# sIncerass/MVLPT

Hardware: AMD Instinct MI355X
Metric: prompt-tuning images/sec (fwd+bwd), ViT-B/16 bs=256, 1/2/4/8 MI355X (higher is better)
Workload: dtype fp16; 1 GPU; BASELINE configs[1]: MVLPT coop head, ViT-B/16, 100 classes (caltech101 token table), n_ctx=16 n_vpt=0, text L=77, class token middle; text_positions_evaluated=77, step_pipelining=True, grad_precision=split_grad, layernorm_folding=both towers, residual_stream=packed fp16 + byte (image tower without prompts / backward), cu_partition=none (towers share every compute unit), per_gpu_batch=256, global_batch=256, parallelism=dp1, text_tower=replicated per GPU

## Files before the change

### include/mvlpt_hip.h

```cpp
#ifndef MVLPT_HIP_H
#define MVLPT_HIP_H
#include <stdint.h>
#ifdef __cplusplus
extern "C" {
#endif

typedef void* mvlpt_stream_t;

enum { MVLPT_DT_F32 = 0, MVLPT_DT_F16 = 1, MVLPT_DT_BF16 = 2 };
enum { MVLPT_LABEL_INT64 = 0, MVLPT_LABEL_PROB_F32 = 1 };
enum { MVLPT_ERR_ARG = -1, MVLPT_ERR_HIP = -2, MVLPT_ERR_STATE = -3, MVLPT_ERR_UNSUPPORTED = -4 };

typedef struct MvlptArch {
  int image_resolution, patch_size, vision_width, vision_layers, vision_heads;
  int context_length, text_width, text_layers, text_heads;
  int embed_dim;
  int compute_dtype;
} MvlptArch;

enum { MVLPT_PREC_FAST = 0, MVLPT_PREC_SPLIT_GRAD = 1, MVLPT_PREC_SPLIT_ALL = 2 };

int mvlpt_create(const MvlptArch* arch, void** handle);
int mvlpt_set_precision(void* handle, int mode);
int mvlpt_set_ln_fold(void* handle, int mode, int min_rows);
// ... 21 lines not shown
                   const int32_t* layout, const int32_t* eot, int C, int L, float* feat_out, int save_for_bwd,
                   mvlpt_stream_t stream);
int mvlpt_text_fwd_grouped(void* handle, const float* prefix, const float* suffix, const float* ctx, int n_ctx, const int32_t* layout,
                           const int32_t* eot, int G, int C, int L, float* feat_out, int save_for_bwd, mvlpt_stream_t stream);
int mvlpt_text_fwd_ranged(void* handle, const float* prefix, const float* suffix, const float* ctx, int n_ctx, const int32_t* layout,
                          const int32_t* eot, const int32_t* class_lo, const int32_t* class_hi, int G, int C, int L, float* feat_out,
                          int save_for_bwd, mvlpt_stream_t stream);
int mvlpt_text_bwd(void* handle, const float* dfeat, float* dctx, mvlpt_stream_t stream);
int mvlpt_text_workspace_bytes(void* handle, int C_total, int L, int save_for_bwd, int64_t* out);

enum { MVLPT_TEXT_MIN_L = 3 };
int mvlpt_text_encode_tokens(void* handle, const int32_t* ids, int ld, int S, int L, float* feat_out, mvlpt_stream_t stream);
int mvlpt_text_ensemble(const float* feats, int T, int C, int e, float* out, mvlpt_stream_t stream);

int mvlpt_logits_fwd(void* handle, const float* img_feat, const float* txt_feat, float logit_scale_exp, const int32_t* task_lo,
                     const int32_t* task_hi, int B, int C, float* logits, mvlpt_stream_t stream);
int mvlpt_logits_bwd(void* handle, const float* dlogits, float* dimg, float* dtxt, mvlpt_stream_t stream);
int mvlpt_logits_grouped_fwd(void* handle, const float* img, const float* txt, float logit_scale_exp, int G, int C, float* logits,
                             mvlpt_stream_t stream);
int mvlpt_logits_grouped_bwd(void* handle, const float* dlogits, float* dtxt, mvlpt_stream_t stream);
int mvlpt_logits_ranged_fwd(void* handle, const float* img, const float* txt, float logit_scale_exp, const int32_t* class_lo,
                            const int32_t* class_hi, int G, int C, float* logits, mvlpt_stream_t stream);
int mvlpt_logits_ranged_bwd(void* handle, const float* dlogits, float* dtxt, float* dimg, mvlpt_stream_t stream);

int mvlpt_cross_entropy(void* handle, const float* logits, const void* labels, int label_kind, int B, int C, float* loss,
                        float* dlogits, float* ncorrect, mvlpt_stream_t stream);

int mvlpt_op_gemm(int dtype, int epi, const void* A, const void* Bt, int M, int N, int K, const float* bias, const void* aux,
                  const float* resid, void* out, void* out2, mvlpt_stream_t stream);
int mvlpt_op_gemm_ex(int dtype, int epi, const void* A, const void* Bt, int M, int N, int K, const float* bias, const void* aux,
                     const float* resid, void* out, void* out2, int a_split, int lda, int ldo, int ldb, int w8_exp, int out_lo8,
                     mvlpt_stream_t stream);
enum { MVLPT_GEMM_BT_128x128_R2 = 1, MVLPT_GEMM_BT_128x128_R4 = 2, MVLPT_GEMM_BT_256x128_R3 = 3, MVLPT_GEMM_BT_256x256_R2 = 4,
       MVLPT_GEMM_PHASED = 5, MVLPT_GEMM_PC = 6, MVLPT_GEMM_PCP = 7 };
int mvlpt_op_gemm_route(int dtype, int epi, int a_split, int M, int N, int K, int fold_ntp, mvlpt_stream_t stream, int* tile_m,
                        int* tile_n, int* ring);
int mvlpt_op_gemm_split(int dtype, int epi, const void* A, const void* Bt, int M, int N, int K, const float* bias, const void* aux,
                        const float* resid, void* out, void* out2, mvlpt_stream_t stream);
int mvlpt_op_layernorm_fwd_split(int out_dtype, const float* x, const float* gamma, const float* beta, void* y, int rows, int d,
                                 mvlpt_stream_t stream);
int mvlpt_op_layernorm_bwd_split(int dtype, const void* dy, const float* x, const float* gamma, const float* resid, float* out32,
                                 void* out16, int rows, int d, mvlpt_stream_t stream);
int mvlpt_op_attention32_fwd(int dtype, const void* qkv, void* out, float* lse, int N, int L, int H, int causal, int q_rows,
                             mvlpt_stream_t stream);
int mvlpt_op_attention32_bwd(int dtype, const void* qkv, const void* out, const void* dout, const float* lse, float* delta,
                             void* dqkv, int N, int L, int H, int causal, mvlpt_stream_t stream);
int mvlpt_op_pack_weight_mixed(int dtype, const float* w32, int rows, int cols, int transposed, void* out, int* w8_exp,
                               mvlpt_stream_t stream);
int mvlpt_op_gemm_mixed(int dtype, int epi, const void* A, const void* Bt, int ldb, int w8_exp, int M, int N, int K, const float* bias,
                        const void* aux, const float* resid, void* out, void* out2, mvlpt_stream_t stream);
int mvlpt_op_cast_mixed(int dtype, const float* in, void* out, int64_t rows, int d, mvlpt_stream_t stream);
int mvlpt_op_fold_vectors(int dtype, const void* W16, int ld, const float* gamma, const float* beta, const float* b, float* colsum,
                          float* bias2, int N, int K, mvlpt_stream_t stream);
int mvlpt_op_gemm_ln_producer(int dtype, const void* A, int a_split, const void* Bt, int ldb, int w8_exp, int M, int N, int K,
                              const float* bias, const float* resid, const float* gamma, int x16_split, float* out32, void* x16,
                              float* part, int ntp, int* nt, mvlpt_stream_t stream);
int mvlpt_op_gemm_folded(int dtype, int epi, const void* A16, int a_split, const void* Bt, int ldb, int w8_exp, int M, int N, int K,
                         const float* colsum, const float* bias2, const float* part, int ntp, int nt, void* out, void* out2,
                         mvlpt_stream_t stream);
int mvlpt_op_fold_weight(const void* W16, int ld, const float* gamma, void* Wg16, int ldg, float* colsum, int N, int K,
                         mvlpt_stream_t stream);
int mvlpt_op_respk_pack(const float* x, void* hi, uint8_t* lo, float* part, int ntp, int rows, int d, mvlpt_stream_t stream);
int mvlpt_op_assemble_packed(const float* patch_emb, const float* cls, const float* pos, const float* ln_g, const float* ln_b, void* hi,
                             uint8_t* lo, float* part, int ntp, int batch, int grid2, int d, mvlpt_stream_t stream);
int mvlpt_op_respk_unpack(const void* hi, const uint8_t* lo, int row_mul, float* out, int rows, int d, mvlpt_stream_t stream);
int mvlpt_op_gemm_residp(const void* A, const void* Bt, int ldb, int M, int N, int K, const float* bias, const void* hi_in,
                         const uint8_t* lo_in, void* hi_out, uint8_t* lo_out, float* part, int ntp, int* nt, mvlpt_stream_t stream);
int mvlpt_op_layernorm_fwd_mixed(int out_dtype, const float* x, const float* gamma, const float* beta, void* y, int rows, int d,
                                 mvlpt_stream_t stream);
int mvlpt_op_layernorm_bwd_mixed(int dtype, const void* dy, const float* x, const float* gamma, const float* resid, float* out32,
                                 void* out16, int rows, int d, mvlpt_stream_t stream);
int mvlpt_op_attention32_fwd_mixed(int dtype, const void* qkv, void* out, float* lse, int N, int L, int H, int causal, int q_rows,
                                   mvlpt_stream_t stream);
int mvlpt_op_attention32_bwd_mixed(int dtype, const void* qkv, const void* out, const void* dout, const float* lse, float* delta,
                                   void* dqkv, int N, int L, int H, int causal, mvlpt_stream_t stream);
int mvlpt_op_layernorm_fwd(int out_dtype, const float* x, const float* gamma, const float* beta, void* y, int rows, int d,
                           mvlpt_stream_t stream);
int mvlpt_op_layernorm_bwd(int dtype, const void* dy, const float* x, const float* gamma, const float* resid, float* out32,
                           void* out16, int rows, int d, mvlpt_stream_t stream);
int mvlpt_op_attention_fwd(int dtype, const void* qkv, void* out, float* lse, int N, int L, int H, int causal,
                           mvlpt_stream_t stream);
int mvlpt_op_attention_bwd(int dtype, const void* qkv, const void* out, const void* dout, const float* lse, float* delta,
                           void* dqkv, int N, int L, int H, int causal, mvlpt_stream_t stream);
int mvlpt_op_cast(int dtype, const float* in, void* out, int64_t n, mvlpt_stream_t stream);
int mvlpt_op_assemble_prompts_grouped(const float* prefix, const float* suffix, const float* ctx, int n_ctx, const int32_t* layout,
                                      const float* pos, float* x, int G, int C, int L, int d, mvlpt_stream_t stream);
int mvlpt_op_gather_ctx_grad_grouped(const float* dx, const int32_t* ctx_pos, int G, int C, int L, int d, int n_ctx, float* dctx,
                                     mvlpt_stream_t stream);
int mvlpt_op_assemble_prompts_ranged(const float* prefix, const float* suffix, const float* ctx, int n_ctx, const int32_t* layout,
                                     const float* pos, float* x, const int32_t* class_lo, const int32_t* class_hi, int G, int C, int L,
                                     int d, mvlpt_stream_t stream);
int mvlpt_op_gather_ctx_grad_ranged(const float* dx, const int32_t* ctx_pos, const int32_t* class_lo, const int32_t* class_hi, int G, int C,
                                    int L, int d, int n_ctx, float* dctx, mvlpt_stream_t stream);

int mvlpt_op_embed_tokens(const float* emb, const float* pos, const int32_t* ids, int ld, float* x, int S, int L, int d,
                          mvlpt_stream_t stream);
int mvlpt_op_ensemble_features(const float* feats, float* out, int T, int C, int e, mvlpt_stream_t stream);
int mvlpt_op_normalize_rows(const float* x, float* xn, float* norm, int rows, int d, mvlpt_stream_t stream);
int mvlpt_op_sgemm_bt(const float* A, const float* Bt, float* C, int M, int N, int K, const float* alpha_dev, mvlpt_stream_t stream);
int mvlpt_op_grad_scale(const float* v, int64_t n, float target, float* scale_dev, mvlpt_stream_t stream);
int mvlpt_op_reduce_prompt_rows(int dtype, float* dx32, void* dx16, int B, int L, int d, int row0, int n, float* out,
                                const float* scale_dev, int zero_after, int split16, const float* vmask, mvlpt_stream_t stream);
int mvlpt_op_gather_ctx_grad(const float* dx, const int32_t* ctx_pos, int C, int L, int d, int n_ctx, int per_class, float* dctx,
                             const float* scale_dev, mvlpt_stream_t stream);
int mvlpt_op_attention_bwd_cls(int dtype, const void* qkv, const void* o_cls, const void* do_cls, const float* lse, void* dqkv, int N,
                               int L, int H, mvlpt_stream_t stream);
int mvlpt_op_copy_rows(const void* src, void* dst, const int32_t* idx, int rows, int row_bytes, int scatter, mvlpt_stream_t stream);
int mvlpt_op_overwrite_rows(const float* rows, int n, float* x, int B, int L, int d, const float* vmask, mvlpt_stream_t stream);
int mvlpt_op_assemble_tokens(const float* patch_emb, const float* cls, const float* pos, const float* ln_g, const float* ln_b,
                             const float* vpt, int n_vpt, const float* vmask, float* x, int B, int G2, int d, mvlpt_stream_t stream);
int mvlpt_op_assemble_prompts(const float* prefix, const float* suffix, const float* ctx, int ctx_per_class, int n_ctx,
                              const int32_t* layout, const float* pos, const int32_t* eot, float* x, int32_t* ctx_pos, int32_t* eot_rows,
                              int C, int L, int d, mvlpt_stream_t stream);

typedef struct MvlptImageDesc {
  int64_t offset;
  int32_t height, width;
  int32_t crop_top, crop_left, crop_height, crop_width;
  int32_t resize_height, resize_width;
  int32_t out_top, out_left;
  int32_t flip;
  int32_t reserved;
} MvlptImageDesc;
int mvlpt_preprocess(void* handle, const uint8_t* src, int64_t src_bytes, const MvlptImageDesc* descs, int B, int out_h, int out_w,
                     const float* mean, const float* std, void* out, int out_dtype, uint8_t* out_u8, mvlpt_stream_t stream);

typedef struct MvlptKernelStat {
  char name[32];
  int64_t launches;
  double ms;
  double flops;
  double bytes;
  double busy_ms;
  double flops_executed;
} MvlptKernelStat;
int mvlpt_profile_begin(void* handle, int all_kernels);
int mvlpt_profile_pause(void* handle, int paused);
int mvlpt_profile_end(void* handle, MvlptKernelStat* stats, int max_stats);

#ifdef __cplusplus
}
#endif
#endif
```

### mvlpt_amd/_lib.py

```python
from __future__ import annotations

import ctypes as C
import os

import torch

_HERE = os.path.dirname(os.path.abspath(__file__))
LIB_PATH = os.environ.get("MVLPT_HIP_LIB") or os.path.join(_HERE, "libmvlpt_hip.so")

DT_F32, DT_F16, DT_BF16 = 0, 1, 2
LABEL_INT64, LABEL_PROB_F32 = 0, 1
EPI_STORE16, EPI_GELU, EPI_RESID32, EPI_GELUBWD, EPI_STORE32, EPI_GELU_SPLIT, EPI_GELUBWD_SPLIT, EPI_STORE_SPLIT = 0, 1, 2, 3, 4, 5, 6, 7
GEMM_BT_128x128_R2, GEMM_BT_128x128_R4, GEMM_BT_256x128_R3, GEMM_BT_256x256_R2, GEMM_PHASED, GEMM_PC, GEMM_PCP = 1, 2, 3, 4, 5, 6, 7
PREC_FAST, PREC_SPLIT_GRAD, PREC_SPLIT_ALL = 0, 1, 2
TEXT_MIN_L = 3


class MvlptArch(C.Structure):
    _fields_ = [(n, C.c_int) for n in (
        "image_resolution", "patch_size", "vision_width", "vision_layers", "vision_heads",
        "context_length", "text_width", "text_layers", "text_heads", "embed_dim", "compute_dtype")]


class MvlptKernelStat(C.Structure):
    _fields_ = [("name", C.c_char * 32), ("launches", C.c_int64), ("ms", C.c_double),
                ("flops", C.c_double), ("bytes", C.c_double), ("busy_ms", C.c_double), ("flops_executed", C.c_double)]


class MvlptImageDesc(C.Structure):
    _fields_ = [("offset", C.c_int64)] + [(n, C.c_int32) for n in (
        "height", "width", "crop_top", "crop_left", "crop_height", "crop_width", "resize_height", "resize_width",
        "out_top", "out_left", "flip", "reserved")]


_vp, _i, _f = C.c_void_p, C.c_int, C.c_float

SIGNATURES = {
    "mvlpt_create": (_i, [C.POINTER(MvlptArch), C.POINTER(_vp)]),
    "mvlpt_destroy": (_i, [_vp]),
    "mvlpt_set_precision": (_i, [_vp, _i]),
    "mvlpt_trim": (_i, [_vp]),
    "mvlpt_debug_checksums": (_i, [_vp, _i, C.POINTER(C.c_uint64), _i]),
    "mvlpt_set_ln_fold": (_i, [_vp, _i, _i]),
    "mvlpt_set_resid_packed": (_i, [_vp, _i]),
    "mvlpt_set_vpt_dropout": (_i, [_vp, _vp, _i, _i, _i, _i]),
    "mvlpt_last_error": (C.c_char_p, [_vp]),
    "mvlpt_version": (C.c_char_p, []),
    "mvlpt_stream_create_cus": (_i, [_i, _i, C.POINTER(_vp)]),
    "mvlpt_stream_destroy": (_i, [_vp]),
    "mvlpt_stream_cus": (_i, [_vp]),
    "mvlpt_load_frozen": (_i, [_vp, C.c_char_p, _vp, _i, C.POINTER(C.c_int64), _i, _vp]),
    "mvlpt_frozen_ready": (_i, [_vp]),
    "mvlpt_image_fwd": (_i, [_vp, _vp, _i, _vp, _vp, _i, _i, _i, _vp, _i, _vp]),
    "mvlpt_image_bwd": (_i, [_vp, _vp, _vp, _vp, _vp]),
    "mvlpt_text_fwd": (_i, [_vp, _vp, _vp, _vp, _i, _i, _vp, _vp, _i, _i, _vp, _i, _vp]),
    "mvlpt_text_bwd": (_i, [_vp, _vp, _vp, _vp]),
    "mvlpt_text_fwd_grouped": (_i, [_vp, _vp, _vp, _vp, _i, _vp, _vp, _i, _i, _i, _vp, _i, _vp]),
    "mvlpt_text_fwd_ranged": (_i, [_vp, _vp, _vp, _vp, _i, _vp, _vp, _vp, _vp, _i, _i, _i, _vp, _i, _vp]),
    "mvlpt_text_workspace_bytes": (_i, [_vp, _i, _i, _i, C.POINTER(C.c_int64)]),
    "mvlpt_text_encode_tokens": (_i, [_vp, _vp, _i, _i, _i, _vp, _vp]),
    "mvlpt_text_ensemble": (_i, [_vp, _i, _i, _i, _vp, _vp]),
    "mvlpt_logits_fwd": (_i, [_vp, _vp, _vp, _f, _vp, _vp, _i, _i, _vp, _vp]),
    "mvlpt_logits_bwd": (_i, [_vp, _vp, _vp, _vp, _vp]),
    "mvlpt_logits_grouped_fwd": (_i, [_vp, _vp, _vp, _f, _i, _i, _vp, _vp]),
    "mvlpt_logits_grouped_bwd": (_i, [_vp, _vp, _vp, _vp]),
    "mvlpt_logits_ranged_fwd": (_i, [_vp, _vp, _vp, _f, _vp, _vp, _i, _i, _vp, _vp]),
    "mvlpt_logits_ranged_bwd": (_i, [_vp, _vp, _vp, _vp, _vp]),
    "mvlpt_cross_entropy": (_i, [_vp, _vp, _vp, _i, _i, _i, _vp, _vp, _vp, _vp]),
    "mvlpt_op_gemm": (_i, [_i, _i, _vp, _vp, _i, _i, _i, _vp, _vp, _vp, _vp, _vp, _vp]),
    "mvlpt_op_gemm_ex": (_i, [_i, _i, _vp, _vp, _i, _i, _i, _vp, _vp, _vp, _vp, _vp, _i, _i, _i, _i, _i, _i, _vp]),
    "mvlpt_op_gemm_route": (_i, [_i, _i, _i, _i, _i, _i, _i, _vp, C.POINTER(_i), C.POINTER(_i), C.POINTER(_i)]),
    "mvlpt_op_gemm_split": (_i, [_i, _i, _vp, _vp, _i, _i, _i, _vp, _vp, _vp, _vp, _vp, _vp]),
    "mvlpt_op_layernorm_fwd_split": (_i, [_i, _vp, _vp, _vp, _vp, _i, _i, _vp]),
    "mvlpt_op_layernorm_bwd_split": (_i, [_i, _vp, _vp, _vp, _vp, _vp, _vp, _i, _i, _vp]),
    "mvlpt_op_attention32_fwd": (_i, [_i, _vp, _vp, _vp, _i, _i, _i, _i, _i, _vp]),
    "mvlpt_op_attention32_bwd": (_i, [_i, _vp, _vp, _vp, _vp, _vp, _vp, _i, _i, _i, _i, _vp]),
    "mvlpt_op_pack_weight_mixed": (_i, [_i, _vp, _i, _i, _i, _vp, C.POINTER(C.c_int), _vp]),
    "mvlpt_op_gemm_mixed": (_i, [_i, _i, _vp, _vp, _i, _i, _i, _i, _i, _vp, _vp, _vp, _vp, _vp, _vp]),
    "mvlpt_op_cast_mixed": (_i, [_i, _vp, _vp, C.c_int64, _i, _vp]),
    "mvlpt_op_fold_vectors": (_i, [_i, _vp, _i, _vp, _vp, _vp, _vp, _vp, _i, _i, _vp]),
    "mvlpt_op_gemm_ln_producer": (_i, [_i, _vp, _i, _vp, _i, _i, _i, _i, _i, _vp, _vp, _vp, _i, _vp, _vp, _vp, _i, C.POINTER(C.c_int), _vp]),
    "mvlpt_op_gemm_folded": (_i, [_i, _i, _vp, _i, _vp, _i, _i, _i, _i, _i, _vp, _vp, _vp, _i, _i, _vp, _vp, _vp]),
    "mvlpt_op_fold_weight": (_i, [_vp, _i, _vp, _vp, _i, _vp, _i, _i, _vp]),
    "mvlpt_op_respk_pack": (_i, [_vp, _vp, _vp, _vp, _i, _i, _i, _vp]),
    "mvlpt_op_assemble_packed": (_i, [_vp, _vp, _vp, _vp, _vp, _vp, _vp, _vp, _i, _i, _i, _i, _vp]),
    "mvlpt_op_respk_unpack": (_i, [_vp, _vp, _i, _vp, _i, _i, _vp]),
    "mvlpt_op_gemm_residp": (_i, [_vp, _vp, _i, _i, _i, _i, _vp, _vp, _vp, _vp, _vp, _vp, _i, C.POINTER(C.c_int), _vp]),
    "mvlpt_op_layernorm_fwd_mixed": (_i, [_i, _vp, _vp, _vp, _vp, _i, _i, _vp]),
    "mvlpt_op_layernorm_bwd_mixed": (_i, [_i, _vp, _vp, _vp, _vp, _vp, _vp, _i, _i, _vp]),
    "mvlpt_op_attention32_fwd_mixed": (_i, [_i, _vp, _vp, _vp, _i, _i, _i, _i, _i, _vp]),
    "mvlpt_op_attention32_bwd_mixed": (_i, [_i, _vp, _vp, _vp, _vp, _vp, _vp, _i, _i, _i, _i, _vp]),
    "mvlpt_op_layernorm_fwd": (_i, [_i, _vp, _vp, _vp, _vp, _i, _i, _vp]),
    "mvlpt_op_layernorm_bwd": (_i, [_i, _vp, _vp, _vp, _vp, _vp, _vp, _i, _i, _vp]),
    "mvlpt_op_attention_fwd": (_i, [_i, _vp, _vp, _vp, _i, _i, _i, _i, _vp]),
    "mvlpt_op_attention_bwd": (_i, [_i, _vp, _vp, _vp, _vp, _vp, _vp, _i, _i, _i, _i, _vp]),
    "mvlpt_op_cast": (_i, [_i, _vp, _vp, C.c_int64, _vp]),
    "mvlpt_op_assemble_prompts_grouped": (_i, [_vp, _vp, _vp, _i, _vp, _vp, _vp, _i, _i, _i, _i, _vp]),
    "mvlpt_op_gather_ctx_grad_grouped": (_i, [_vp, _vp, _i, _i, _i, _i, _i, _vp, _vp]),
    "mvlpt_op_assemble_prompts_ranged": (_i, [_vp, _vp, _vp, _i, _vp, _vp, _vp, _vp, _vp, _i, _i, _i, _i, _vp]),
    "mvlpt_op_gather_ctx_grad_ranged": (_i, [_vp, _vp, _vp, _vp, _i, _i, _i, _i, _i, _vp, _vp]),
    "mvlpt_op_embed_tokens": (_i, [_vp, _vp, _vp, _i, _vp, _i, _i, _i, _vp]),
    "mvlpt_op_ensemble_features": (_i, [_vp, _vp, _i, _i, _i, _vp]),
    "mvlpt_op_normalize_rows": (_i, [_vp, _vp, _vp, _i, _i, _vp]),
    "mvlpt_op_sgemm_bt": (_i, [_vp, _vp, _vp, _i, _i, _i, _vp, _vp]),
    "mvlpt_op_grad_scale": (_i, [_vp, C.c_int64, _f, _vp, _vp]),
    "mvlpt_op_reduce_prompt_rows": (_i, [_i, _vp, _vp, _i, _i, _i, _i, _i, _vp, _vp, _i, _i, _vp, _vp]),
    "mvlpt_op_gather_ctx_grad": (_i, [_vp, _vp, _i, _i, _i, _i, _i, _vp, _vp, _vp]),
    "mvlpt_op_attention_bwd_cls": (_i, [_i, _vp, _vp, _vp, _vp, _vp, _i, _i, _i, _vp]),
    "mvlpt_op_copy_rows": (_i, [_vp, _vp, _vp, _i, _i, _i, _vp]),
    "mvlpt_op_overwrite_rows": (_i, [_vp, _i, _vp, _i, _i, _i, _vp, _vp]),
    "mvlpt_op_assemble_tokens": (_i, [_vp, _vp, _vp, _vp, _vp, _vp, _i, _vp, _vp, _i, _i, _i, _vp]),
    "mvlpt_op_assemble_prompts": (_i, [_vp, _vp, _vp, _i, _i, _vp, _vp, _vp, _vp, _vp, _vp, _i, _i, _i, _vp]),
    "mvlpt_preprocess": (_i, [_vp, _vp, C.c_int64, C.POINTER(MvlptImageDesc), _i, _i, _i, C.POINTER(_f), C.POINTER(_f), _vp, _i, _vp, _vp]),
    "mvlpt_profile_begin": (_i, [_vp, _i]),
    "mvlpt_profile_pause": (_i, [_vp, _i]),
    "mvlpt_profile_end": (_i, [_vp, C.POINTER(MvlptKernelStat), _i]),
}


def load_library(path: str = LIB_PATH) -> C.CDLL:
    if not os.path.isfile(path):
        raise ImportError(
            f"{path} not found: build the HIP extension first (`make` at the repo root, or "
            "`__graft_entry__.build()`); mvlpt_amd has no CPU fallback.")
    lib = C.CDLL(path)
    for name, (res, args) in SIGNATURES.items():
        fn = getattr(lib, name)
        fn.restype, fn.argtypes = res, args
    return lib


lib = load_library()


def last_error(handle=None) -> str:
    msg = lib.mvlpt_last_error(handle)
    return msg.decode() if msg else ""


def check(rc: int, handle=None, what: str = "") -> None:
    if rc != 0:
        raise RuntimeError(f"libmvlpt_hip {what} failed (code {rc}): {last_error(handle) or last_error(None)}")
```

### mvlpt_amd/csrc/attention.hip

```cpp
#include <hip/hip_ext.h>
#include "attn_common.h"

namespace mvlpt {

constexpr int ATT_MAX_NKT = 38;
int attn_max_len() { return ATT_MAX_NKT * 16; }

template <typename T, int NKT, bool CAUSAL>
__global__ __launch_bounds__(256) void attn_fwd_kernel(AttnArgs a) {
  extern __shared__ __attribute__((aligned(16))) char smem[];
  using v8 = typename Vec<T>::v8;
  using v4 = typename Vec<T>::v4;
  constexpr int LP = NKT * 16;
  constexpr int BLK = NKT < 16 ? NKT : 16;
  constexpr bool PRELOAD = NKT <= 16;
  char* sK = smem;
  char* sV = smem + LP * 128;
  const int L = a.L, H = a.H, d = H * 64;
  const int n = blockIdx.x / H, h = blockIdx.x % H;
  const size_t ld = (size_t)3 * d;
  const T* base = (const T*)a.qkv + (size_t)n * L * ld + h * 64;
  const int lane = threadIdx.x & 63, wave = __builtin_amdgcn_readfirstlane(threadIdx.x >> 6);
  const int fr = lane & 15, fg = lane >> 4;
  const int nqt = a.q_rows > 0 ? ((a.q_rows < L ? a.q_rows : L) + 15) >> 4 : (L + 15) >> 4;
// ... 480 lines not shown
template <typename T>
__device__ __forceinline__ float cls_dot16(const float* g16, const typename Vec<T>::v8& a0, const typename Vec<T>::v8& a1) {
  float s = 0.f;
#pragma unroll
  for (int e = 0; e < 8; ++e) { s = fmaf(g16[e], to_f32<T>(a0[e]), s); s = fmaf(g16[e + 8], to_f32<T>(a1[e]), s); }
  s += __shfl_xor(s, 1, 64); s += __shfl_xor(s, 2, 64);
  return s;
}
template <typename T>
__global__ __launch_bounds__(256) void attn_bwd_cls_kernel(const T* __restrict__ qkv, const T* __restrict__ o_cls,
                                                           const T* __restrict__ do_cls, const float* __restrict__ lse,
                                                           T* __restrict__ dqkv, int N, int L, int H) {
  using v8 = typename Vec<T>::v8;
  __shared__ float sq[64], sdo[64], red[4][64];
  const int n = blockIdx.x / H, h = blockIdx.x % H, d = H * 64, tid = threadIdx.x;
  const size_t ld = (size_t)3 * d;
  const T* base = qkv + (size_t)n * L * ld + h * 64;
  T* gbase = dqkv + (size_t)n * L * ld + h * 64;
  if (tid < 64) {
    sq[tid] = to_f32<T>(base[tid]);
    sdo[tid] = to_f32<T>(do_cls[(size_t)n * d + h * 64 + tid]);
  }
  __syncthreads();
  const float l0 = lse[((size_t)n * H + h) * L];
  const int lane = tid & 63, wave = tid >> 6, kg = lane >> 2, ch = lane & 3;
  float q16[16], g16[16], dqa[16];
#pragma unroll
  for (int e = 0; e < 16; ++e) { q16[e] = sq[ch * 16 + e]; g16[e] = sdo[ch * 16 + e]; dqa[e] = 0.f; }
  const T* op = o_cls + (size_t)n * d + h * 64 + ch * 16;
  const float delta = cls_dot16<T>(g16, *(const v8*)op, *(const v8*)(op + 8));
  for (int j0 = wave * 16; j0 < L; j0 += 64) {
    const int j = j0 + kg;
    const int jc = j < L ? j : L - 1;
    const T* kp = base + (size_t)jc * ld + d + ch * 16;
    const v8 k0 = *(const v8*)kp, k1 = *(const v8*)(kp + 8);
    const v8 v0 = *(const v8*)(kp + d), v1 = *(const v8*)(kp + d + 8);
    float k16[16], sdot = 0.f;
#pragma unroll
    for (int e = 0; e < 8; ++e) { k16[e] = to_f32<T>(k0[e]); k16[e + 8] = to_f32<T>(k1[e]); }
    const float dp = cls_dot16<T>(g16, v0, v1);
#pragma unroll
    for (int e = 0; e < 16; ++e) sdot += q16[e] * k16[e];
    sdot += __shfl_xor(sdot, 1, 64); sdot += __shfl_xor(sdot, 2, 64);
    const float pj = j < L ? __expf(sdot * 0.125f - l0) : 0.f;
    const float ds = pj * (dp - delta) * 0.125f;
    v8 wk[2], wv[2], wz[2];
#pragma unroll
    for (int e = 0; e < 16; ++e) {
      dqa[e] += ds * k16[e];
      wk[e >> 3][e & 7] = from_f32<T>(ds * q16[e]);
      wv[e >> 3][e & 7] = from_f32<T>(pj * g16[e]);
      wz[e >> 3][e & 7] = from_f32<T>(0.f);
    }
    if (j < L) {
      T* gp = gbase + (size_t)j * ld + ch * 16;
      if (j > 0) { *(v8*)gp = wz[0]; *(v8*)(gp + 8) = wz[1]; }
      *(v8*)(gp + d) = wk[0]; *(v8*)(gp + d + 8) = wk[1];
      *(v8*)(gp + 2 * d) = wv[0]; *(v8*)(gp + 2 * d + 8) = wv[1];
    }
  }
#pragma unroll
  for (int e = 0; e < 16; ++e) {
    float v = dqa[e];
    v += __shfl_xor(v, 4, 64); v += __shfl_xor(v, 8, 64); v += __shfl_xor(v, 16, 64); v += __shfl_xor(v, 32, 64);
    if (kg == 0) red[wave][ch * 16 + e] = v;
  }
  __syncthreads();
  if (tid < 64) gbase[tid] = from_f32<T>(red[0][tid] + red[1][tid] + red[2][tid] + red[3][tid]);
}

hipError_t launch_attn_bwd_cls(int dtype, const void* qkv, const void* o_cls, const void* do_cls, const float* lse, void* dqkv,
                               int N, int L, int H, hipStream_t s) {
  if (N <= 0 || L <= 0 || H <= 0) return hipErrorInvalidValue;
  if (dtype == DT_F16)
    hipLaunchKernelGGL(attn_bwd_cls_kernel<f16>, dim3(N * H), dim3(256), 0, s, (const f16*)qkv, (const f16*)o_cls, (const f16*)do_cls, lse,
                       (f16*)dqkv, N, L, H);
  else if (dtype == DT_BF16)
    hipLaunchKernelGGL(attn_bwd_cls_kernel<bf16>, dim3(N * H), dim3(256), 0, s, (const bf16*)qkv, (const bf16*)o_cls, (const bf16*)do_cls,
                       lse, (bf16*)dqkv, N, L, H);
  else return hipErrorInvalidValue;
  return hipGetLastError();
}

static thread_local hipEvent_t t_ev_a = nullptr, t_ev_b = nullptr;
template <typename T, int NKT, bool CAUSAL>
static hipError_t fwd_t(const AttnArgs& a, hipStream_t s) {
  constexpr int LP = NKT * 16;
  constexpr int lds = 2 * LP * 128;
  static bool set = false;
  if (!set) { hipFuncSetAttribute((const void*)attn_fwd_kernel<T, NKT, CAUSAL>, hipFuncAttributeMaxDynamicSharedMemorySize, lds); set = true; }
  hipExtLaunchKernelGGL((attn_fwd_kernel<T, NKT, CAUSAL>), dim3(a.N * a.H), dim3(256), lds, s, t_ev_a, t_ev_b, 0, a);
  return hipGetLastError();
}
template <typename T, int NKT, bool CAUSAL>
static hipError_t bwd_t(const AttnBwdArgs& a, hipStream_t s) {
  constexpr int LP = NKT * 16;
  constexpr int lds_a = 2 * LP * 128;
  constexpr int lds_b = 2 * LP * 128 + 2 * LP * 4;
  static bool set = false;
  if (!set) {
    hipFuncSetAttribute((const void*)attn_bwd_dq_kernel<T, NKT, CAUSAL>, hipFuncAttributeMaxDynamicSharedMemorySize, lds_a);
    hipFuncSetAttribute((const void*)attn_bwd_dkv_kernel<T, NKT, CAUSAL>, hipFuncAttributeMaxDynamicSharedMemorySize, lds_b);
    set = true;
  }
  hipLaunchKernelGGL((attn_bwd_dq_kernel<T, NKT, CAUSAL>), dim3(a.N * a.H), dim3(256), lds_a, s, a);
  hipError_t e = hipGetLastError();
  if (e != hipSuccess) return e;
  hipLaunchKernelGGL((attn_bwd_dkv_kernel<T, NKT, CAUSAL>), dim3(a.N * a.H), dim3(256), lds_b, s, a);
  return hipGetLastError();
}

#define MVLPT_NKT_SWITCH(FN, ARGS)                                  \
  switch (nkt) {                                                    \
    case 2: return FN<T, 2, CAUSAL> ARGS;                           \
    case 4: return FN<T, 4, CAUSAL> ARGS;                           \
    case 6: return FN<T, 6, CAUSAL> ARGS;                           \
    case 8: return FN<T, 8, CAUSAL> ARGS;                           \
    case 10: return FN<T, 10, CAUSAL> ARGS;                         \
    case 12: return FN<T, 12, CAUSAL> ARGS;                         \
    case 14: return FN<T, 14, CAUSAL> ARGS;                         \
    case 16: return FN<T, 16, CAUSAL> ARGS;                         \
  }                                                                 \
  if constexpr (!CAUSAL) {    \
    if (nkt == 18) return FN<T, 18, CAUSAL> ARGS;                   \
    if (nkt == 38) return FN<T, 38, CAUSAL> ARGS;                   \
  }                                                                 \
  return hipErrorInvalidValue;

template <typename T, bool CAUSAL> static hipError_t fwd_n(int nkt, const AttnArgs& a, hipStream_t s) {
  if constexpr (!CAUSAL) { if (nkt == 13) return fwd_t<T, 13, CAUSAL>(a, s); }
  MVLPT_NKT_SWITCH(fwd_t, (a, s))
}
template <typename T, bool CAUSAL> static hipError_t bwd_n(int nkt, const AttnBwdArgs& a, hipStream_t s) { MVLPT_NKT_SWITCH(bwd_t, (a, s)) }

static int nkt_for(int L) {
  int t = (L + 15) / 16; t += t & 1;
  if (t > 18) return 38;
  return t < 2 ? 2 : t;
}

static bool use_stream(int L) { return L > 256; }

hipError_t launch_attn_fwd(int dtype, const AttnArgs& a_, hipStream_t s, hipEvent_t ea, hipEvent_t eb) {
  t_ev_a = ea; t_ev_b = eb;
  AttnArgs a = a_;
  a.flags = 3;
  if (a.L <= 0 || a.L > attn_max_len() || a.N <= 0) return hipErrorInvalidValue;
  if (use_stream(a.L)) return launch_attn_fwd_stream(dtype, a, s);
  if (!a.causal && a.q_rows <= 0 && (a.L + 15) / 16 == PNT && (dtype == DT_F16 || dtype == DT_BF16)) {
    const int total = a.N * a.H, cus = stream_cus(s);
    if (total >= 2 * cus) {
      static bool set = false;
      if (!set) {
        hipFuncSetAttribute((const void*)attn_fwdp_kernel<f16>, hipFuncAttributeMaxDynamicSharedMemorySize, PLDS);
        hipFuncSetAttribute((const void*)attn_fwdp_kernel<bf16>, hipFuncAttributeMaxDynamicSharedMemorySize, PLDS);
        set = true;
      }
      if (dtype == DT_F16) hipExtLaunchKernelGGL((attn_fwdp_kernel<f16>), dim3(cus), dim3(PNW * 64), PLDS, s, ea, eb, 0, a, total);
      else hipExtLaunchKernelGGL((attn_fwdp_kernel<bf16>), dim3(cus), dim3(PNW * 64), PLDS, s, ea, eb, 0, a, total);
      return hipGetLastError();
    }
  }
  const int nkt = !a.causal && (a.L + 15) / 16 == 13 ? 13 : nkt_for(a.L);
  if (dtype == DT_F16) return a.causal ? fwd_n<f16, true>(nkt, a, s) : fwd_n<f16, false>(nkt, a, s);
  if (dtype == DT_BF16) return a.causal ? fwd_n<bf16, true>(nkt, a, s) : fwd_n<bf16, false>(nkt, a, s);
  return hipErrorInvalidValue;
// ... 12 lines not shown
```

### mvlpt_amd/csrc/attention32.hip

```cpp
#include "attn_common.h"

namespace mvlpt {

#ifdef MVLPT_ATTN_TRACE
constexpr int ATR_MAX = 256;
#define MVLPT_ATR(p) do { if (a.trace && blockIdx.x == 1024 && lane == 0 && atr_n < ATR_MAX) \
    a.trace[wave * ATR_MAX + atr_n++] = ((long long)(p) << 56) | ((long long)__builtin_amdgcn_s_memtime() & 0xffffffffffffffLL); } while (0)
#define MVLPT_ATRB(p) do { if (a.trace && blockIdx.x == 5 && blockIdx.y == (gridDim.y >> 1) && lane == 0 && atr_n < ATR_MAX) \
    a.trace[wave * ATR_MAX + atr_n++] = ((long long)(p) << 56) | ((long long)__builtin_amdgcn_s_memtime() & 0xffffffffffffffLL); } while (0)
#else
#define MVLPT_ATR(p) do { } while (0)
#define MVLPT_ATRB(p) do { } while (0)
#endif

namespace {
constexpr int CH = 64;
constexpr int XIMG = CH * 128;
constexpr float SCALE = 0.125f;

template <typename T>
__device__ __forceinline__ void store_pair4(T* p, size_t lo_off, f32x4 v) {
  typename Vec<T>::v4 hi, lo;
#pragma unroll
  for (int e = 0; e < 4; ++e) { T h, l; split16<T>(v[e], h, l); hi[e] = h; lo[e] = l; }
// ... 1094 lines not shown
static bool attn32_resident(int L, int causal) { return !causal && L <= RROWS; }

static int attn32_nw(int rows) {
  const int pad8 = (rows + 255) / 256 * 256, pad4 = (rows + 127) / 128 * 128;
  return pad8 * 8 <= pad4 * 9 ? 8 : 4;
}
template <typename K>
static void set_lds(K kernel, int bytes) { (void)hipFuncSetAttribute((const void*)kernel, hipFuncAttributeMaxDynamicSharedMemorySize, bytes); }

template <typename T, bool CAUSAL, int NW>
static hipError_t fwd_x(const Attn32Args& a, hipStream_t s) {
  const int lq = a.q_rows > 0 ? (a.q_rows < a.L ? a.q_rows : a.L) : a.L;
  const int nqc = (lq + NW * 32 - 1) / (NW * 32);
  constexpr int lds = 8 * XIMG;
  static bool set = false;
  if (!set) { set_lds(attn32x_fwd_kernel<T, CAUSAL, NW>, lds); set = true; }
  hipLaunchKernelGGL((attn32x_fwd_kernel<T, CAUSAL, NW>), dim3(stream_grid(a.N * a.H, nqc)), dim3(NW * 64), lds, s, a, nqc);
  return hipGetLastError();
}
template <typename T, bool CAUSAL, int NW>
static hipError_t bwd_x(const Attn32BwdArgs& a, hipStream_t s) {
  const int nc = (a.L + NW * 32 - 1) / (NW * 32), lpad = (a.L + CH - 1) / CH * CH;
  constexpr int lds = 8 * XIMG;
  const int lds_kv = lds + 8 * lpad;
  static int set = 0;
  if (set < lds_kv) {
    set_lds(attn32x_dq_kernel<T, CAUSAL, NW>, lds); set_lds(attn32x_dkv_kernel<T, CAUSAL, NW>, lds_kv);
    set_lds(attn32x_bwd_fused_kernel<T, CAUSAL, NW>, lds_kv); set = lds_kv;
  }
  const dim3 grid(stream_grid(a.N * a.H, nc)), block(NW * 64);
  if (nc == 1) {
    hipLaunchKernelGGL((attn32x_bwd_fused_kernel<T, CAUSAL, NW>), grid, block, lds_kv, s, a, lpad);
    return hipGetLastError();
  }
  hipLaunchKernelGGL((attn32x_dq_kernel<T, CAUSAL, NW>), grid, block, lds, s, a, nc);
  hipLaunchKernelGGL((attn32x_dkv_kernel<T, CAUSAL, NW>), grid, block, lds_kv, s, a, nc, lpad);
  return hipGetLastError();
}

template <typename T>
static hipError_t fwd_t(const Attn32Args& a, hipStream_t s) {
  if (a.L <= SROWS) {
    dim3 grid(a.H, a.N), block(SNT * 64);
    if (a.causal) hipLaunchKernelGGL((attn32t_fwd_kernel<T, true>), grid, block, 0, s, a);
    else hipLaunchKernelGGL((attn32t_fwd_kernel<T, false>), grid, block, 0, s, a);
    return hipGetLastError();
  }
  if (attn32_resident(a.L, a.causal)) {
    const int total = a.N * a.H, cus = stream_cus(s);
    if (a.q_rows <= 0 && total >= 2 * cus) {
      static bool setp = false;
      if (!setp) { set_lds(attn32p_fwd_kernel<T>, RLDS_P); setp = true; }
      hipLaunchKernelGGL((attn32p_fwd_kernel<T>), dim3(cus), dim3(RNW * 64), RLDS_P, s, a, total);
      return hipGetLastError();
    }
    static bool set = false;
    if (!set) { set_lds(attn32r_fwd_kernel<T>, RLDS); set = true; }
    hipLaunchKernelGGL((attn32r_fwd_kernel<T>), dim3(a.H, a.N), dim3(RNW * 64), RLDS, s, a);
    return hipGetLastError();
  }
  const int lq = a.q_rows > 0 ? (a.q_rows < a.L ? a.q_rows : a.L) : a.L;
  if (attn32_nw(lq) == 8) return a.causal ? fwd_x<T, true, 8>(a, s) : fwd_x<T, false, 8>(a, s);
  return a.causal ? fwd_x<T, true, 4>(a, s) : fwd_x<T, false, 4>(a, s);
}
template <typename T>
static hipError_t bwd_t(const Attn32BwdArgs& a, hipStream_t s) {
  if (a.L <= SROWS) {
    dim3 grid(a.H, a.N), block(SNT * 64);
    if (a.causal) hipLaunchKernelGGL((attn32t_bwd_kernel<T, true>), grid, block, 0, s, a);
    else hipLaunchKernelGGL((attn32t_bwd_kernel<T, false>), grid, block, 0, s, a);
    return hipGetLastError();
  }
  if (attn32_resident(a.L, a.causal)) {
    static bool set = false;
    if (!set) { set_lds(attn32r_bwd_kernel<T>, RLDS_BWD); set = true; }
    hipLaunchKernelGGL((attn32r_bwd_kernel<T>), dim3(a.H, a.N), dim3(RNW * 64), RLDS_BWD, s, a);
    return hipGetLastError();
  }
  if (a.L > 8192) return hipErrorInvalidValue;
  if (attn32_nw(a.L) == 8) return a.causal ? bwd_x<T, true, 8>(a, s) : bwd_x<T, false, 8>(a, s);
  return a.causal ? bwd_x<T, true, 4>(a, s) : bwd_x<T, false, 4>(a, s);
}

hipError_t launch_attn32_fwd(int dtype, const Attn32Args& a, hipStream_t s) {
  if (a.L <= 0 || a.N <= 0 || a.H <= 0 || !a.qkv_split || !a.out_split) return hipErrorInvalidValue;
  if (dtype == DT_F16) return fwd_t<f16>(a, s);
  if (dtype == DT_BF16) return fwd_t<bf16>(a, s);
  return hipErrorInvalidValue;
}
hipError_t launch_attn32_bwd(int dtype, const Attn32BwdArgs& a, hipStream_t s) {
  if (a.L <= 0 || a.N <= 0 || a.H <= 0 || !a.qkv_split || !a.out_split || !a.dout_split || !a.lse || !a.delta || !a.dqkv_split)
    return hipErrorInvalidValue;
  if (dtype == DT_F16) return bwd_t<f16>(a, s);
  if (dtype == DT_BF16) return bwd_t<bf16>(a, s);
  return hipErrorInvalidValue;
}

}
```

### mvlpt_amd/csrc/engine.hip

```cpp
#include <hip/hip_runtime.h>

#include <cmath>
#include <cstdio>
#include <algorithm>
#include <array>
#include <map>
#include <cstring>
#include <mutex>
#include <string>
#include <vector>

#include "../../include/mvlpt_hip.h"
#include "kernels.h"

using namespace mvlpt;


namespace {
struct StreamPart { hipStream_t s; int cus; };
std::mutex g_part_mu;
std::vector<StreamPart> g_parts;
int device_cus() {
  static int cus = 0;
  if (!cus) {
// ... 32 lines not shown
  }
  hipError_t reserve(size_t bytes) {
    if (bytes <= cap) return hipSuccess;
    size_t got = std::max(bytes, cap + cap / 2);
    void* q = nullptr;
    hipError_t e = hipMalloc(&q, got);
    if (e != hipSuccess && got > bytes) { got = bytes; e = hipMalloc(&q, got); }
    if (e != hipSuccess) return e;
    if (p) retired.push_back(p);
    p = q; cap = got;
    return hipSuccess;
  }
};
struct Bump {
  char* base = nullptr; size_t off = 0, cap = 0;
  template <typename T> T* take(size_t count) {
    size_t bytes = (count * sizeof(T) + 255) & ~(size_t)255;
    T* r = (T*)(base + off); off += bytes; return r;
  }
  void* take_bytes(size_t bytes) { return take<char>(bytes); }
};
static size_t align256(size_t b) { return (b + 255) & ~(size_t)255; }

struct WRef { const void* p; int ld; int e8; };
struct Linear {
  void* w = nullptr; void* wt = nullptr; float* b = nullptr; int out = 0, in = 0;
  int ldw = 0, ldwt = 0, e8 = 0;
  float *fold_s = nullptr, *fold_b = nullptr;
  void* wg = nullptr; float* fold_sg = nullptr;
  WRef fw() const { return WRef{w, ldw, e8}; }
  WRef fwg() const { return WRef{wg, in, 0}; }
  WRef bw() const { return WRef{wt, ldwt, e8}; }
};
struct LNp { float* g = nullptr; float* b = nullptr; };
struct Block { LNp ln1, ln2; Linear qkv, o, fc, pr; };
struct TowerW { int width = 0, layers = 0, heads = 0; std::vector<Block> blocks; };

struct TowerState {
  bool valid = false, saved = false, causal = false;
  bool exact = false;
  int wide_pitch = 0;
  int xs = 0;
  int N = 0, L = 0, d = 0, H = 0, layers = 0;
  std::vector<float*> x;
  std::vector<void*> qkv, attn, u;
  std::vector<float*> lse;
  void *h16 = nullptr, *a16 = nullptr;
  float* dx32 = nullptr; void *dx16 = nullptr, *du16 = nullptr, *dO16 = nullptr, *dqkv16 = nullptr; float* dh32 = nullptr;
  float* delta = nullptr; float* scale_dev = nullptr;
  std::vector<char> skip;
  bool fold = false;
  float* part[2] = {nullptr, nullptr};
  int nt[2] = {0, 0}, ntp[2] = {0, 0};
};
constexpr int FOLD_NTP = 8;

enum ProfClass { PC_GEMM = 0, PC_ATTN_FWD, PC_ATTN_BWD, PC_LN_FWD, PC_LN_BWD, PC_GLUE, PC_HEAD, PC_ATTN_FWD_IMG, PC_COUNT };
static const char* kProfNames[PC_COUNT] = {"gemm_bt", "attention_fwd", "attention_bwd", "layernorm_fwd", "layernorm_bwd",
                                           "glue", "head_logits_ce", "attention_fwd_image"};
struct ProfRec { int cls; hipEvent_t a, b; double flops, bytes, flops_exec; int M = 0, N = 0, K = 0, epi = -1, split = 0, fold = 0; };

struct Engine {
  MvlptArch arch{};
  int dt = DT_F16;
  int prec_mode = MVLPT_PREC_SPLIT_GRAD;
  int fold_mode = 2;
  int fold_min_rows = 1024;
  bool fold_ready = false;
  int resid_packed = 1;
  const float* vpt_mask = nullptr;
  int vpt_mask_layers = 0, vpt_mask_B = 0, vpt_mask_n = 0, vpt_mask_d = 0;
  const float* v_mask = nullptr;
  bool lo8 = true;
  std::string err;
  TowerW vis, txt;
  void* conv_w = nullptr; int Kp = 0; float* cls_emb = nullptr; float* vpos = nullptr; LNp ln_pre, ln_post;
  float *vproj = nullptr, *vproj_t = nullptr;
  float* tpos = nullptr; LNp ln_final; float *tproj = nullptr, *tproj_t = nullptr;
  float* tok_emb = nullptr; int vocab = 0;
  std::vector<void*> owned;
  DevBuf vis_ws, txt_ws, head_ws, ce_ws, tmp, pp_ws;
  TowerState vs, ts;
  int vB = 0, v_nvpt = 0, v_ndeep = 0; float* cls32 = nullptr; float* dcls32 = nullptr;
  float* xc32 = nullptr; void *ac16 = nullptr, *hc16 = nullptr, *gc16 = nullptr;
  bool v_cls_last = false; float *xcm32 = nullptr, *xco32 = nullptr, *dxc32 = nullptr, *dhc32 = nullptr;
  void *uc16 = nullptr, *duc16 = nullptr, *dxc16 = nullptr, *dOc16 = nullptr;
  int tC = 0, tL = 0, t_nctx = 0, t_per_class = 0; int32_t* eot_rows = nullptr; int32_t* ctx_pos = nullptr;
  int t_groups = 0, t_gC = 0;
  bool t_ranged = false; const int32_t *t_rlo = nullptr, *t_rstart = nullptr;
  std::vector<int32_t> t_range_host, h_range_host;
  std::vector<int32_t> t_ids_host;
  bool t_eot_last = false; float *txc32 = nullptr, *txm32 = nullptr, *txo32 = nullptr, *tdxc32 = nullptr, *tdhc32 = nullptr;
  void *tac16 = nullptr, *thc16 = nullptr, *tgc16 = nullptr, *tuc16 = nullptr, *tduc16 = nullptr, *tdxc16 = nullptr, *tdOc16 = nullptr;
  float* eot32 = nullptr; float* deot32 = nullptr;
  int hB = 0, hC = 0; float h_scale = 0.f; const int32_t *h_lo = nullptr, *h_hi = nullptr;
  bool h_grouped = false;
  bool h_ranged = false; int hS = 0; const int32_t *h_rlo = nullptr, *h_rstart = nullptr, *h_rgrp = nullptr;
  float *imn = nullptr, *txn = nullptr, *inorm = nullptr, *tnorm = nullptr;
  unsigned long long* dbg_ck = nullptr; int dbg_ck_n = 0; bool dbg_ck_on = false;
  bool prof_on = false, prof_all = false; std::vector<ProfRec> prof; std::vector<hipEvent_t> ev_pool; size_t ev_used = 0;
};

thread_local std::string g_create_err;

int fail(Engine* E, int code, const std::string& msg) { if (E) E->err = msg; else g_create_err = msg; return code; }
int hipfail(Engine* E, hipError_t e, const char* what) {
  return fail(E, MVLPT_ERR_HIP, std::string(what) + ": " + hipGetErrorString(e));
}
#define HIPCHK(E, call) do { hipError_t _e = (call); if (_e != hipSuccess) return hipfail((E), _e, #call); } while (0)

struct ProfScope {
  Engine* E; hipStream_t s; bool on = false; hipEvent_t b{};
  ProfScope(Engine* E_, hipStream_t s_, int cls, double flops, double bytes) : E(E_), s(s_) {
    if (!E || !E->prof_on || !E->prof_all) return;
    if (E->ev_used + 2 > E->ev_pool.size()) {
      if (E->ev_pool.size() >= 65536) return;
      for (int i = 0; i < 512; ++i) { hipEvent_t ev; if (hipEventCreate(&ev) != hipSuccess) return; E->ev_pool.push_back(ev); }
    }
    hipEvent_t a = E->ev_pool[E->ev_used++]; b = E->ev_pool[E->ev_used++];
    (void)hipEventRecord(a, s);
    E->prof.push_back(ProfRec{cls, a, b, flops, bytes, flops});
    on = true;
  }
  ~ProfScope() { if (on) (void)hipEventRecord(b, s); }
};

constexpr int DBG_CK_MAX = 256;
static void dbg_ck(Engine* E, const void* p, size_t bytes, hipStream_t s) {
  if (!E->dbg_ck_on || !E->dbg_ck || E->dbg_ck_n >= DBG_CK_MAX) return;
  (void)launch_checksum(p, bytes, E->dbg_ck + E->dbg_ck_n++, s);
}

static hipError_t attn_fwd_timed(Engine* E, const AttnArgs& a, double flops, double bytes, hipStream_t s) {
  hipEvent_t ea = nullptr, eb = nullptr;
  if (E && E->prof_on && !E->prof_all) {
    if (E->ev_used + 2 > E->ev_pool.size() && E->ev_pool.size() < 65536)
      for (int i = 0; i < 512; ++i) { hipEvent_t ev; if (hipEventCreate(&ev) != hipSuccess) break; E->ev_pool.push_back(ev); }
    if (E->ev_used + 2 <= E->ev_pool.size()) {
      ea = E->ev_pool[E->ev_used++]; eb = E->ev_pool[E->ev_used++];
      E->prof.push_back(ProfRec{PC_ATTN_FWD_IMG, ea, eb, flops, bytes, flops});
    }
  }
  return launch_attn_fwd(E->dt, a, s, ea, eb);
}

struct Fold {
  const float* ln_gamma = nullptr; void* ln_x16 = nullptr; int ln_split = 0; float* ln_part = nullptr; int ln_ntp = 0;
  const float* fold_part = nullptr; const float* fold_colsum = nullptr; int fold_ntp = 0, fold_nt = 0;
  const void* rp_hi_in = nullptr; const uint8_t* rp_lo_in = nullptr; uint8_t* rp_lo_out = nullptr;
};
hipError_t gemm(Engine* E, int epi, const void* A, WRef Bt, int M, int N, int K, const float* bias, const void* aux,
                const float* resid, void* out, void* out2, hipStream_t s, int dtype = -1, int a_split = 0, const Fold* f = nullptr,
                int lda = 0, int ldo = 0) {
  GemmArgs g{A, Bt.p, M, N, K, bias, aux, resid, out, out2};
  g.a_split = a_split; g.ldb = Bt.ld; g.w8_exp = Bt.e8; g.lda = lda; g.ldo = ldo;
  if (f) {
    g.ln_gamma = f->ln_gamma; g.ln_x16 = f->ln_x16; g.ln_split = f->ln_split; g.ln_part = f->ln_part; g.ln_ntp = f->ln_ntp;
    g.fold_part = f->fold_part; g.fold_colsum = f->fold_colsum; g.fold_ntp = f->fold_ntp; g.fold_nt = f->fold_nt;
    g.rp_hi_in = f->rp_hi_in; g.rp_lo_in = f->rp_lo_in; g.rp_lo_out = f->rp_lo_out;
  }
  g.out_lo8 = (a_split == 2 && (epi == EPI_GELU_SPLIT || epi == EPI_GELUBWD_SPLIT)) ? 1 : 0;
  const int dt = dtype >= 0 ? dtype : E->dt;
  const double ob = (epi == EPI_RESIDP_LN) ? 6.0 : (epi == EPI_RESID32) ? 8.0 : (epi == EPI_RESID32_LN) ? 8.0 + 2.0 * (a_split ? 1.5 : 1.0) : ((epi == EPI_STORE32 || epi == EPI_STORE_SPLIT) ? 4.0 : ((epi == EPI_GELUBWD || epi == EPI_GELU_SPLIT) ? 4.0 :
                    (epi == EPI_GELUBWD_SPLIT ? 6.0 : 2.0)));
  hipEvent_t ea = nullptr, eb = nullptr;
  if (E && E->prof_on) {
    if (E->ev_used + 2 > E->ev_pool.size() && E->ev_pool.size() < 65536)
// ... 506 lines not shown
  const MvlptArch& A = E->arch;
  const int dv = A.vision_width, dtw = A.text_width, e = A.embed_dim;
  const int G2 = (A.image_resolution / A.patch_size) * (A.image_resolution / A.patch_size);
  auto is1 = [&](int r) { return ndim == 1 && shape[0] == r; };
  auto is2 = [&](int r, int c) { return ndim == 2 && shape[0] == r && shape[1] == c; };
  int rc = 0;
  const char* vb = "visual.transformer.resblocks.";
  const char* tb = "transformer.resblocks.";
  if (nm.rfind(vb, 0) == 0 || nm.rfind(tb, 0) == 0) {
    const bool isv = nm.rfind(vb, 0) == 0;
    int layer; const char* tail;
    if (!parse_block_name(name + strlen(isv ? vb : tb), &layer, &tail)) return fail(E, MVLPT_ERR_ARG, "malformed block name: " + nm);
    rc = load_block_tensor(E, isv ? E->vis : E->txt, layer, tail, p32, shape, ndim, s);
  } else if (nm == "visual.conv1.weight") {
    if (!(ndim == 4 && shape[0] == dv && shape[1] == 3 && shape[2] == A.patch_size && shape[3] == A.patch_size))
      return fail(E, MVLPT_ERR_ARG, "shape mismatch: " + nm);
    void* w = nullptr;
    HIPCHK(E, hipMalloc(&w, (size_t)dv * E->Kp * 2)); E->owned.push_back(w);
    HIPCHK(E, launch_pack_weight(E->dt, p32, w, dv, 3 * A.patch_size * A.patch_size, E->Kp, s));
    E->conv_w = w;
  } else if (nm == "visual.class_embedding") { if (!is1(dv)) return fail(E, MVLPT_ERR_ARG, "shape mismatch: " + nm); rc = upload_f32(E, p32, n, &E->cls_emb, s);
  } else if (nm == "visual.positional_embedding") { if (!is2(G2 + 1, dv)) return fail(E, MVLPT_ERR_ARG, "shape mismatch: " + nm); rc = upload_f32(E, p32, n, &E->vpos, s);
  } else if (nm == "visual.ln_pre.weight") { if (!is1(dv)) return fail(E, MVLPT_ERR_ARG, "shape mismatch: " + nm); rc = upload_f32(E, p32, n, &E->ln_pre.g, s);
  } else if (nm == "visual.ln_pre.bias") { if (!is1(dv)) return fail(E, MVLPT_ERR_ARG, "shape mismatch: " + nm); rc = upload_f32(E, p32, n, &E->ln_pre.b, s);
  } else if (nm == "visual.ln_post.weight") { if (!is1(dv)) return fail(E, MVLPT_ERR_ARG, "shape mismatch: " + nm); rc = upload_f32(E, p32, n, &E->ln_post.g, s);
  } else if (nm == "visual.ln_post.bias") { if (!is1(dv)) return fail(E, MVLPT_ERR_ARG, "shape mismatch: " + nm); rc = upload_f32(E, p32, n, &E->ln_post.b, s);
  } else if (nm == "visual.proj") {
    if (!is2(dv, e)) return fail(E, MVLPT_ERR_ARG, "shape mismatch: " + nm);
    void *w = nullptr, *wt = nullptr;
    HIPCHK(E, hipMalloc(&w, n * 4)); E->owned.push_back(w);
    HIPCHK(E, hipMalloc(&wt, n * 4)); E->owned.push_back(wt);
    HIPCHK(E, launch_pack_weight(DT_F32, p32, w, dv, e, e, s));
    HIPCHK(E, launch_pack_weight_t(DT_F32, p32, wt, dv, e, s));
    E->vproj = (float*)w; E->vproj_t = (float*)wt;
  } else if (nm == "positional_embedding") { if (!is2(A.context_length, dtw)) return fail(E, MVLPT_ERR_ARG, "shape mismatch: " + nm); rc = upload_f32(E, p32, n, &E->tpos, s);
  } else if (nm == "ln_final.weight") { if (!is1(dtw)) return fail(E, MVLPT_ERR_ARG, "shape mismatch: " + nm); rc = upload_f32(E, p32, n, &E->ln_final.g, s);
  } else if (nm == "ln_final.bias") { if (!is1(dtw)) return fail(E, MVLPT_ERR_ARG, "shape mismatch: " + nm); rc = upload_f32(E, p32, n, &E->ln_final.b, s);
  } else if (is_tok) {
    if (!(ndim == 2 && shape[0] > 0 && shape[0] <= INT32_MAX && shape[1] == dtw)) return fail(E, MVLPT_ERR_ARG, "shape mismatch: " + nm);
    E->vocab = 0;
    rc = upload_f32(E, p32, n, &E->tok_emb, s);
    if (!rc) E->vocab = (int)shape[0];
  } else if (nm == "text_projection") {
    if (!is2(dtw, e)) return fail(E, MVLPT_ERR_ARG, "shape mismatch: " + nm);
    void *w = nullptr, *wt = nullptr;
    HIPCHK(E, hipMalloc(&w, n * 4)); E->owned.push_back(w);
    HIPCHK(E, hipMalloc(&wt, n * 4)); E->owned.push_back(wt);
    HIPCHK(E, launch_pack_weight(DT_F32, p32, w, dtw, e, e, s));
    HIPCHK(E, launch_pack_weight_t(DT_F32, p32, wt, dtw, e, s));
    E->tproj = (float*)w; E->tproj_t = (float*)wt;
  } else {
    return fail(E, MVLPT_ERR_ARG, "unknown frozen tensor name: " + nm);
  }
  if (rc) return rc;
  if (dtype != MVLPT_DT_F32) HIPCHK(E, hipStreamSynchronize(s));
  return 0;
}

int mvlpt_frozen_ready(void* h) {
  Engine* E = (Engine*)h;
  if (!E) return MVLPT_ERR_ARG;
  const char* m = first_missing(E);
  if (m) return fail(E, MVLPT_ERR_STATE, std::string("frozen tensor not loaded: ") + m);
  return 0;
}

int mvlpt_image_fwd(void* h, const void* image, int image_dtype, const float* vpt, const float* vpt_deep, int n_vpt, int n_deep,
                    int B, float* feat_out, int save_for_bwd, mvlpt_stream_t stream) {
  Engine* E = (Engine*)h;
  if (!E || !image || !feat_out || B <= 0) return fail(E, MVLPT_ERR_ARG, "image_fwd: null/invalid argument");
  if (int rc = mvlpt_frozen_ready(h)) return rc;
  if ((n_vpt > 0) != (vpt != nullptr)) return fail(E, MVLPT_ERR_ARG, "image_fwd: vpt pointer and n_vpt disagree");
  if ((n_deep > 0) != (vpt_deep != nullptr) || (n_deep > 0 && n_vpt <= 0)) return fail(E, MVLPT_ERR_ARG, "image_fwd: deep prompts need vpt");
  hipStream_t s = (hipStream_t)stream;
  const MvlptArch& A = E->arch;
  const int G = A.image_resolution / A.patch_size, G2 = G * G, dv = A.vision_width, e = A.embed_dim;
  const int Lv = 1 + n_vpt + G2;
  if (Lv > attn_max_len()) return fail(E, MVLPT_ERR_UNSUPPORTED, "image_fwd: sequence length > 256 not supported yet");
  const bool save = save_for_bwd != 0;
  const bool exact = E->prec_mode == MVLPT_PREC_SPLIT_ALL || (E->prec_mode == MVLPT_PREC_SPLIT_GRAD && save);
  const size_t X = exact ? 2 : 1;
  const size_t npatch = (size_t)B * G2;
  size_t need = tower_bytes(E->vis, B, Lv, save, exact) + align256(npatch * E->Kp * 2) + align256(npatch * dv * 4) +
                7 * align256((size_t)B * dv * 4) + 4 * align256((size_t)B * dv * 2 * X) + 3 * align256((size_t)B * dv * 8 * X) + 4096;
  E->vs.valid = false;
  HIPCHK(E, E->vis_ws.reserve(need));
  Bump bp; bp.base = (char*)E->vis_ws.p; bp.cap = E->vis_ws.cap;
  void* patches = bp.take_bytes(npatch * E->Kp * 2);
  float* pe = bp.take<float>(npatch * dv);
  E->cls32 = bp.take<float>((size_t)B * dv);
  E->dcls32 = bp.take<float>((size_t)B * dv);
  E->xc32 = bp.take<float>((size_t)B * dv);
  E->ac16 = bp.take_bytes((size_t)B * dv * 2 * X); E->hc16 = bp.take_bytes((size_t)B * dv * 2 * X);
  E->gc16 = bp.take_bytes((size_t)B * dv * 4 * 2 * X);
  E->xcm32 = bp.take<float>((size_t)B * dv); E->xco32 = bp.take<float>((size_t)B * dv);
  E->dxc32 = bp.take<float>((size_t)B * dv); E->dhc32 = bp.take<float>((size_t)B * dv);
  E->dxc16 = bp.take_bytes((size_t)B * dv * 2 * X); E->dOc16 = bp.take_bytes((size_t)B * dv * 2 * X);
  E->uc16 = bp.take_bytes((size_t)B * dv * 4 * 2); E->duc16 = bp.take_bytes((size_t)B * dv * 4 * 2 * X);
  E->v_cls_last = false;
  carve_tower(bp, E->vis, E->vs, B, Lv, save, false, exact, split_kind(E));
  TowerState& st = E->vs;
  E->vB = B; E->v_nvpt = n_vpt; E->v_ndeep = n_deep;
  st.fold = E->fold_mode >= 1 && (size_t)B * Lv >= (size_t)E->fold_min_rows && dv >= 256;
  if (st.fold) if (int rc = prepare_fold(E, s)) return rc;

  const float* const masks = E->vpt_mask;
  const int mask_layers = E->vpt_mask_layers, mask_B = E->vpt_mask_B, mask_n = E->vpt_mask_n;
  E->vpt_mask = nullptr; E->vpt_mask_layers = 0; E->v_mask = nullptr;
  if (masks && (n_vpt <= 0 || mask_layers < 1 + n_deep || mask_B != B || mask_n != n_vpt))
    return fail(E, MVLPT_ERR_ARG, "image_fwd: the prompt dropout masks do not match this forward (layers >= 1 + n_deep, batch, n_vpt)");
  E->v_mask = masks;
  auto vmask = [&](int l) -> const float* { return masks ? masks + (size_t)l * B * n_vpt * dv : nullptr; };
  { ProfScope ps(E, s, PC_GLUE, 0, (double)npatch * E->Kp * 6.0);
    HIPCHK(E, launch_patchify(E->dt, image, image_dtype, patches, B, A.image_resolution, A.patch_size, E->Kp, s)); }
  if (E->dbg_ck_on) { E->dbg_ck_n = 0; if (E->dbg_ck) (void)hipMemsetAsync(E->dbg_ck, 0, DBG_CK_MAX * sizeof(unsigned long long), s); }
  dbg_ck(E, patches, (size_t)npatch * E->Kp * 2, s);
  HIPCHK(E, gemm(E, EPI_STORE32, patches, WRef{E->conv_w, 0, 0}, (int)npatch, dv, E->Kp, nullptr, nullptr, nullptr, pe, nullptr, s));
  dbg_ck(E, pe, (size_t)npatch * dv * 4, s);
  const int nt_d = dv / 128, ntp_d = (nt_d + 1) & ~1;
  const bool packed = E->resid_packed && E->dt == DT_F16 && !save && !exact && st.fold && n_vpt == 0 && dv % 128 == 0 &&
                      ntp_d <= FOLD_NTP && E->vis.blocks[0].qkv.wg != nullptr;
  void* const xhi = st.x[0];
  uint8_t* const xlo = (uint8_t*)st.x[0] + (size_t)B * Lv * dv * 2;
  if (packed) {
    ProfScope ps(E, s, PC_GLUE, 0, (double)B * Lv * dv * 7.0);
    HIPCHK(E, launch_assemble_tokens_packed(pe, E->cls_emb, E->vpos, E->ln_pre.g, E->ln_pre.b, xhi, xlo, st.part[0], ntp_d, B, G2, dv, s));
    st.nt[0] = nt_d; st.ntp[0] = ntp_d;
    dbg_ck(E, xhi, (size_t)B * Lv * dv * 3, s); dbg_ck(E, st.part[0], (size_t)B * Lv * ntp_d * 8, s);
  } else {
    ProfScope ps(E, s, PC_GLUE, 0, (double)B * Lv * dv * 8.0);
    HIPCHK(E, launch_assemble_tokens(pe, E->cls_emb, E->vpos, E->ln_pre.g, E->ln_pre.b, vpt, n_vpt, st.x[0], B, G2, dv, s, vmask(0)));
  }
  bool cls_only_last = false;
  bool ln1_ready = packed;
  auto next_foldable = [&](int l) -> const LNp* {
    const int n = l + 1;
    if (!st.fold || n >= E->vis.layers) return nullptr;
    if (n_deep > 0) return nullptr;
    return &E->vis.blocks[n].ln1;
  };
  for (int l = 0; l < E->vis.layers; ++l) {
    if (l > 0 && n_deep > 0) {
      if (l <= n_deep) {
        ProfScope ps(E, s, PC_GLUE, 0, (double)B * n_vpt * dv * 4.0);
        HIPCHK(E, launch_overwrite_rows(vpt_deep + (size_t)(l - 1) * n_vpt * dv, n_vpt, st.x[2 * l], B, Lv, dv, s, vmask(l)));
      } else {
        st.skip[l] = 1;
        if (st.saved) {
          HIPCHK(E, hipMemcpyAsync(st.x[2 * l + 2], st.x[2 * l], (size_t)B * Lv * dv * 4, hipMemcpyDeviceToDevice, s));
        }
        continue;
      }
    }
    if (l == E->vis.layers - 1) { cls_only_last = true; break; }
    if (packed) { if (int rc = block_fwd_packed(E, E->vis, st, l, s)) return rc; continue; }
    bool produced = false;
    if (int rc = block_fwd(E, E->vis, st, l, s, ln1_ready, next_foldable(l), &produced)) return rc;
    ln1_ready = produced;
  }
  if (cls_only_last) {
    const int l = E->vis.layers - 1;
    const Block& Bk = E->vis.blocks[l];
    const int T = B * Lv;
    float* xin = st.x[2 * l];
    float* xmid = save ? E->xcm32 : E->xc32;
    float* xout = save ? E->xco32 : E->xc32;
    E->v_cls_last = save;
    const int xs = st.xs;
    Fold fq;
    if (ln1_ready) fq = fold_consumer(st, 0, Bk.qkv);
    else HIPCHK(E, ln_fwd(E, E->dt, xin, nullptr, 1, Bk.ln1, st.h16, T, dv, s, xs));
    if (packed) fq.fold_colsum = Bk.qkv.fold_sg;
    HIPCHK(E, gemm(E, xs ? EPI_STORE_SPLIT : EPI_STORE16, packed ? xhi : st.h16, packed ? Bk.qkv.fwg() : Bk.qkv.fw(), T, 3 * dv, dv,
                   ln1_ready ? Bk.qkv.fold_b : Bk.qkv.b, nullptr, nullptr, st.qkv[l], nullptr, s, -1, xs, ln1_ready ? &fq : nullptr));
    dbg_ck(E, st.qkv[l], (size_t)T * 3 * dv * 2 * X, s);
    if (xs) {
      if (save) HIPCHK(E, launch_zero(st.attn[l], (size_t)T * dv * 4, s));
      if (int rc = attn32_fwd(E, st, l, 1, s)) return rc;
    } else {
      AttnArgs a{st.qkv[l], st.attn[l], save ? st.lse[l] : nullptr, st.N, st.L, st.H, 0, 1};
      ProfScope ps(E, s, PC_ATTN_FWD, 4.0 * st.L * 64.0 * st.N * st.H, (double)T * dv * 2.0 * 2.0);
      HIPCHK(E, launch_attn_fwd(E->dt, a, s));
    }
    { ProfScope ps(E, s, PC_GLUE, 0, (double)B * dv * 12.0);
      HIPCHK(E, launch_copy_rows_strided(st.attn[l], E->ac16, B, (size_t)Lv * dv * 2 * X, (size_t)dv * 2 * X, (int)(dv * 2 * X), s));
      if (packed) HIPCHK(E, launch_respk_unpack_rows(xhi, xlo, Lv, E->xc32, B, dv, s));
      else HIPCHK(E, launch_copy_rows_strided(xin, E->xc32, B, (size_t)Lv * dv * 4, (size_t)dv * 4, dv * 4, s)); }
    dbg_ck(E, E->ac16, (size_t)B * dv * 2 * X, s); dbg_ck(E, E->xc32, (size_t)B * dv * 4, s);
    HIPCHK(E, gemm(E, EPI_RESID32, E->ac16, Bk.o.fw(), B, dv, dv, Bk.o.b, nullptr, E->xc32, xmid, nullptr, s, -1, xs));
    HIPCHK(E, ln_fwd(E, E->dt, xmid, nullptr, 1, Bk.ln2, E->hc16, B, dv, s, xs));
    HIPCHK(E, gemm(E, xs ? EPI_GELU_SPLIT : EPI_GELU, E->hc16, Bk.fc.fw(), B, 4 * dv, dv, Bk.fc.b, nullptr, nullptr, E->gc16, save ? E->uc16 : nullptr, s, -1, xs));
    HIPCHK(E, gemm(E, EPI_RESID32, E->gc16, Bk.pr.fw(), B, dv, 4 * dv, Bk.pr.b, nullptr, xmid, xout, nullptr, s, -1, xs));
    HIPCHK(E, ln_fwd(E, DT_F32, xout, nullptr, 1, E->ln_post, E->cls32, B, dv, s));
  } else
  HIPCHK(E, ln_fwd(E, DT_F32, st.x[2 * E->vis.layers], nullptr, Lv, E->ln_post, E->cls32, B, dv, s));
  { ProfScope ps(E, s, PC_HEAD, 2.0 * B * e * dv, 4.0 * ((double)B * dv + (double)e * dv + (double)B * e));
    HIPCHK(E, launch_sgemm_bt(E->cls32, E->vproj_t, feat_out, B, e, dv, nullptr, s)); }
  return 0;
}

int mvlpt_image_bwd(void* h, const float* dfeat, float* dvpt, float* dvpt_deep, mvlpt_stream_t stream) {
  Engine* E = (Engine*)h;
  if (!E || !dfeat) return fail(E, MVLPT_ERR_ARG, "image_bwd: null argument");
  TowerState& st = E->vs;
  if (!st.valid || !st.saved) return fail(E, MVLPT_ERR_STATE, "image_bwd: call image_fwd(save_for_bwd=1) first");
  if ((E->v_nvpt > 0 && !dvpt) || (E->v_ndeep > 0 && !dvpt_deep)) return fail(E, MVLPT_ERR_ARG, "image_bwd: missing gradient output");
  hipStream_t s = (hipStream_t)stream;
  const MvlptArch& A = E->arch;
  const int B = E->vB, dv = A.vision_width, e = A.embed_dim, Lv = st.L, n = E->v_nvpt;
  const size_t T = (size_t)B * Lv;
  { ProfScope ps(E, s, PC_GLUE, 0, (double)T * dv * 10.0);
    HIPCHK(E, launch_grad_scale(dfeat, (size_t)B * e, 64.0f, st.scale_dev, s));
    HIPCHK(E, launch_sgemm_bt(dfeat, E->vproj, E->dcls32, B, dv, e, st.scale_dev, s)); }
  { ProfScope ps(E, s, PC_GLUE, 0, (double)T * dv * 4.0);
    HIPCHK(E, launch_zero(st.dx32, T * dv * 4, s)); }
  int l_top = st.layers - 1;
  const int xs = st.xs;
  if (E->v_cls_last) {
    const int l = st.layers - 1;
    const Block& Bk = E->vis.blocks[l];
    const int Ti = (int)T;
    HIPCHK(E, ln_bwd(E, E->dcls32, DT_F32, E->xco32, nullptr, 1, E->ln_post, nullptr, E->dxc32, E->dxc16, B, dv, s, -1, xs));
    HIPCHK(E, gemm(E, xs ? EPI_GELUBWD_SPLIT : EPI_GELUBWD, E->dxc16, Bk.pr.bw(), B, 4 * dv, dv, nullptr, E->uc16, nullptr, E->duc16, nullptr, s, -1, xs));
    HIPCHK(E, gemm(E, EPI_STORE32, E->duc16, Bk.fc.bw(), B, dv, 4 * dv, nullptr, nullptr, nullptr, E->dhc32, nullptr, s, -1, xs));
    HIPCHK(E, ln_bwd(E, E->dhc32, DT_F32, E->xcm32, nullptr, 1, Bk.ln2, E->dxc32, E->dxc32, E->dxc16, B, dv, s, -1, xs));
    HIPCHK(E, gemm(E, xs ? EPI_STORE_SPLIT : EPI_STORE16, E->dxc16, Bk.o.bw(), B, dv, dv, nullptr, nullptr, nullptr, E->dOc16, nullptr, s, -1, xs));
    if (xs) {
      { ProfScope ps(E, s, PC_GLUE, 0, (double)T * dv * 4.0);
        HIPCHK(E, launch_zero(st.dO16, T * dv * 4, s));
        HIPCHK(E, launch_copy_rows_strided(E->dOc16, st.dO16, B, (size_t)dv * 4, (size_t)Lv * dv * 4, dv * 4, s)); }
      if (int rc = attn32_bwd(E, st, l, s)) return rc;
    } else {
      ProfScope ps(E, s, PC_ATTN_BWD, 10.0 * st.L * 64.0 * st.N * st.H, (double)T * dv * 2.0 * 5.0);
      HIPCHK(E, launch_attn_bwd_cls(E->dt, st.qkv[l], E->ac16, E->dOc16, st.lse[l], st.dqkv16, st.N, st.L, st.H, s)); }
    { ProfScope ps(E, s, PC_GLUE, 0, (double)B * dv * 8.0);
      HIPCHK(E, launch_copy_rows_strided(E->dxc32, st.dx32, B, (size_t)dv * 4, (size_t)Lv * dv * 4, dv * 4, s)); }
    HIPCHK(E, gemm(E, EPI_STORE32, st.dqkv16, Bk.qkv.bw(), Ti, dv, 3 * dv, nullptr, nullptr, nullptr, st.dh32, nullptr, s, -1, xs));
    HIPCHK(E, ln_bwd(E, st.dh32, DT_F32, st.x[2 * l], nullptr, 1, Bk.ln1, st.dx32, st.dx32, st.dx16, Ti, dv, s, -1, xs));
    if (l > 0 && E->v_ndeep > 0 && l <= E->v_ndeep) {
      ProfScope ps(E, s, PC_GLUE, 0, (double)B * n * dv * 10.0);
      HIPCHK(E, launch_reduce_prompt_rows(E->dt, st.dx32, st.dx16, B, Lv, dv, 1, n, dvpt_deep + (size_t)(l - 1) * n * dv,
                                          st.scale_dev, 1, s, xs, E->v_mask ? E->v_mask + (size_t)l * B * n * dv : nullptr));
    }
    l_top = l - 1;
  } else {
    HIPCHK(E, ln_bwd(E, E->dcls32, DT_F32, st.x[2 * st.layers], nullptr, Lv, E->ln_post, nullptr, st.dx32, nullptr, B, dv, s));
    { ProfScope ps(E, s, PC_GLUE, 0, (double)T * dv * 6.0);
      if (xs) HIPCHK(E, launch_cast_f32_split(E->dt, st.dx32, st.dx16, T, dv, nullptr, s, xs == 2));
      else HIPCHK(E, launch_cast_f32_to16(E->dt, st.dx32, st.dx16, T * dv, nullptr, s)); }
  }
  for (int l = l_top; l >= 0; --l) {
    if (st.skip[l]) continue;
    if (int rc = block_bwd(E, E->vis, st, l, s)) return rc;
    if (l > 0 && E->v_ndeep > 0 && l <= E->v_ndeep) {
      ProfScope ps(E, s, PC_GLUE, 0, (double)B * n * dv * 10.0);
      HIPCHK(E, launch_reduce_prompt_rows(E->dt, st.dx32, st.dx16, B, Lv, dv, 1, n, dvpt_deep + (size_t)(l - 1) * n * dv,
                                          st.scale_dev, 1, s, xs, E->v_mask ? E->v_mask + (size_t)l * B * n * dv : nullptr));
    }
  }
  if (n > 0) {
    ProfScope ps(E, s, PC_GLUE, 0, (double)B * n * dv * 4.0);
    HIPCHK(E, launch_reduce_prompt_rows(E->dt, st.dx32, st.dx16, B, Lv, dv, 1, n, dvpt, st.scale_dev, 0, s, 0, E->v_mask));
  }
  return 0;
}

static int64_t build_range_table(const int32_t* class_lo, const int32_t* class_hi, int G, int C, std::vector<int32_t>& t) {
  int64_t S = 0;
  for (int g = 0; g < G; ++g) {
    if (class_lo[g] < 0 || class_lo[g] > class_hi[g] || class_hi[g] > C) return -1;
    S += class_hi[g] - class_lo[g];
// ... 18 lines not shown
}
static bool text_exact(const Engine* E) { return E->prec_mode == MVLPT_PREC_SPLIT_ALL || E->prec_mode == MVLPT_PREC_SPLIT_GRAD; }

static int text_fwd_impl(Engine* E, const float* prefix, const float* suffix, const float* ctx, int ctx_per_class, int n_ctx,
                         const int32_t* layout, const int32_t* eot, int G, int Cg, int C, int L, float* feat_out, int save_for_bwd,
                         mvlpt_stream_t stream, bool ranged = false, bool ids = false) {
  if (int rc = mvlpt_frozen_ready(E)) return rc;
  if ((n_ctx > 0) != (ctx != nullptr) || n_ctx < 0 || n_ctx > L - 2) return fail(E, MVLPT_ERR_ARG, "text_fwd: ctx pointer and n_ctx disagree");
  const MvlptArch& A = E->arch;
  if (L > A.context_length) return fail(E, MVLPT_ERR_ARG, "text_fwd: L exceeds context_length");
  if (L > attn_max_len()) return fail(E, MVLPT_ERR_UNSUPPORTED, "text_fwd: L > 256");
  hipStream_t s = (hipStream_t)stream;
  const int dtw = A.text_width, e = A.embed_dim;
  const bool save = save_for_bwd != 0;
  const bool exact = text_exact(E);
  const size_t X = exact ? 2 : 1;
  const size_t ctx_rows = (size_t)(ranged && Cg > C ? Cg : C) * (n_ctx > 0 ? n_ctx : 1);
  const size_t range_ints = ranged ? E->t_range_host.size() : 0;
  const size_t ids_ints = ids ? E->t_ids_host.size() : 0;
  size_t need = text_ws_bytes(E, C, L, save, exact, ctx_rows) + align256(range_ints * 4) + align256(ids_ints * 4);
  E->ts.valid = false;
  HIPCHK(E, E->txt_ws.reserve(need));
  Bump bp; bp.base = (char*)E->txt_ws.p; bp.cap = E->txt_ws.cap;
  E->eot32 = bp.take<float>((size_t)C * dtw);
  E->deot32 = bp.take<float>((size_t)C * dtw);
  E->eot_rows = bp.take<int32_t>(C);
  E->ctx_pos = bp.take<int32_t>(ctx_rows);
  int32_t* range_dev = ranged ? bp.take<int32_t>(range_ints) : nullptr;
  int32_t* ids_dev = ids ? bp.take<int32_t>(ids_ints) : nullptr;
  E->txc32 = bp.take<float>((size_t)C * dtw); E->txm32 = bp.take<float>((size_t)C * dtw); E->txo32 = bp.take<float>((size_t)C * dtw);
  E->tdxc32 = bp.take<float>((size_t)C * dtw); E->tdhc32 = bp.take<float>((size_t)C * dtw);
  E->tac16 = bp.take_bytes((size_t)C * dtw * 2 * X); E->thc16 = bp.take_bytes((size_t)C * dtw * 2 * X);
  E->tdxc16 = bp.take_bytes((size_t)C * dtw * 2 * X); E->tdOc16 = bp.take_bytes((size_t)C * dtw * 2 * X);
  E->tgc16 = bp.take_bytes((size_t)C * dtw * 8 * X); E->tuc16 = bp.take_bytes((size_t)C * dtw * 8); E->tduc16 = bp.take_bytes((size_t)C * dtw * 8 * X);
  E->t_eot_last = false;
  carve_tower(bp, E->txt, E->ts, C, L, save, true, exact, split_kind(E));
  TowerState& st = E->ts;
  E->tC = C; E->tL = L; E->t_nctx = n_ctx; E->t_per_class = ctx_per_class;
  E->t_groups = G; E->t_gC = G > 0 ? Cg : 0;
  E->t_ranged = ranged; E->t_rlo = range_dev; E->t_rstart = ranged ? range_dev + G : nullptr;
  st.fold = E->fold_mode >= 2 && (size_t)C * L >= (size_t)E->fold_min_rows && dtw >= 256;
  if (st.fold) if (int rc = prepare_fold(E, s)) return rc;
  if (ids) {
    ProfScope ps(E, s, PC_GLUE, 0, (double)C * L * dtw * 12.0);
    HIPCHK(E, hipMemcpyAsync(ids_dev, E->t_ids_host.data(), ids_ints * 4, hipMemcpyHostToDevice, s));
    HIPCHK(E, hipMemcpyAsync(E->eot_rows, ids_dev + (size_t)C * L, (size_t)C * 4, hipMemcpyDeviceToDevice, s));
    HIPCHK(E, launch_embed_tokens(E->tok_emb, E->tpos, ids_dev, L, st.x[0], C, L, dtw, s));
  } else
  { ProfScope ps(E, s, PC_GLUE, 0, (double)C * L * dtw * 12.0);
    if (ranged) {
      const int32_t *seq_cls = range_dev + 2 * G + 1, *seq_grp = seq_cls + C;
      HIPCHK(E, hipMemcpyAsync(range_dev, E->t_range_host.data(), range_ints * 4, hipMemcpyHostToDevice, s));
      HIPCHK(E, launch_assemble_prompts_ranged(prefix, suffix, ctx, n_ctx, layout, E->tpos, st.x[0], seq_cls, seq_grp, C, L, dtw, s));
      HIPCHK(E, launch_eot_rows_ranged(eot, E->eot_rows, seq_cls, C, L, s));
      if (save) HIPCHK(E, launch_build_ctx_pos(layout, E->ctx_pos, Cg, L, n_ctx, s));
    } else if (G > 0) {
      HIPCHK(E, launch_assemble_prompts_grouped(prefix, suffix, ctx, n_ctx, layout, E->tpos, st.x[0], G, Cg, L, dtw, s));
      HIPCHK(E, launch_eot_rows_grouped(eot, E->eot_rows, G, Cg, L, s));
      if (save) HIPCHK(E, launch_build_ctx_pos(layout, E->ctx_pos, Cg, L, n_ctx, s));
    } else {
      HIPCHK(E, launch_assemble_prompts(prefix, suffix, ctx, ctx_per_class, n_ctx, layout, E->tpos, st.x[0], C, L, dtw, s));
      HIPCHK(E, launch_eot_rows(eot, E->eot_rows, C, L, s));
      if (save && n_ctx > 0) HIPCHK(E, launch_build_ctx_pos(layout, E->ctx_pos, C, L, n_ctx, s));
    } }
  bool ln1_ready = false;
  for (int l = 0; l + 1 < E->txt.layers; ++l) {
    bool produced = false;
    if (int rc = block_fwd(E, E->txt, st, l, s, ln1_ready, st.fold ? &E->txt.blocks[l + 1].ln1 : nullptr, &produced)) return rc;
    ln1_ready = produced;
  }
  {
    const int l = E->txt.layers - 1;
    const Block& Bk = E->txt.blocks[l];
    const int T = C * L;
    float* xin = st.x[2 * l];
    E->t_eot_last = save;
    const int xs = st.xs;
    Fold fq;
    if (ln1_ready) fq = fold_consumer(st, 0, Bk.qkv);
    else HIPCHK(E, ln_fwd(E, E->dt, xin, nullptr, 1, Bk.ln1, st.h16, T, dtw, s, xs));
    HIPCHK(E, gemm(E, xs ? EPI_STORE_SPLIT : EPI_STORE16, st.h16, Bk.qkv.fw(), T, 3 * dtw, dtw, ln1_ready ? Bk.qkv.fold_b : Bk.qkv.b, nullptr, nullptr, st.qkv[l], nullptr, s, -1, xs,
                   ln1_ready ? &fq : nullptr));
    if (xs) {
      if (int rc = attn32_fwd(E, st, l, 0, s)) return rc;
    } else {
      AttnArgs a{st.qkv[l], st.attn[l], save ? st.lse[l] : nullptr, st.N, st.L, st.H, 1};
      ProfScope ps(E, s, PC_ATTN_FWD, 2.0 * st.L * st.L * 64.0 * st.N * st.H, (double)T * dtw * 2.0 * 4.0);
      HIPCHK(E, launch_attn_fwd(E->dt, a, s));
    }
    { ProfScope ps(E, s, PC_GLUE, 0, (double)C * dtw * 12.0);
      HIPCHK(E, launch_copy_rows(st.attn[l], E->tac16, E->eot_rows, C, (int)(dtw * 2 * X), 0, s));
      HIPCHK(E, launch_copy_rows(xin, E->txc32, E->eot_rows, C, dtw * 4, 0, s)); }
    HIPCHK(E, gemm(E, EPI_RESID32, E->tac16, Bk.o.fw(), C, dtw, dtw, Bk.o.b, nullptr, E->txc32, E->txm32, nullptr, s, -1, xs));
    HIPCHK(E, ln_fwd(E, E->dt, E->txm32, nullptr, 1, Bk.ln2, E->thc16, C, dtw, s, xs));
    HIPCHK(E, gemm(E, xs ? EPI_GELU_SPLIT : EPI_GELU, E->thc16, Bk.fc.fw(), C, 4 * dtw, dtw, Bk.fc.b, nullptr, nullptr, E->tgc16, save ? E->tuc16 : nullptr, s, -1, xs));
    HIPCHK(E, gemm(E, EPI_RESID32, E->tgc16, Bk.pr.fw(), C, dtw, 4 * dtw, Bk.pr.b, nullptr, E->txm32, E->txo32, nullptr, s, -1, xs));
    HIPCHK(E, ln_fwd(E, DT_F32, E->txo32, nullptr, 1, E->ln_final, E->eot32, C, dtw, s));
  }
  { ProfScope ps(E, s, PC_HEAD, 2.0 * C * e * dtw, 4.0 * ((double)C * dtw + (double)e * dtw + (double)C * e));
    HIPCHK(E, launch_sgemm_bt(E->eot32, E->tproj_t, feat_out, C, e, dtw, nullptr, s)); }
  return 0;
}

int mvlpt_text_fwd(void* h, const float* prefix, const float* suffix, const float* ctx, int ctx_per_class, int n_ctx,
                   const int32_t* layout, const int32_t* eot, int C, int L, float* feat_out, int save_for_bwd,
                   mvlpt_stream_t stream) {
  Engine* E = (Engine*)h;
  if (!E || !prefix || !suffix || !layout || !eot || !feat_out || C <= 0 || L <= 0)
    return fail(E, MVLPT_ERR_ARG, "text_fwd: null/invalid argument");
  return text_fwd_impl(E, prefix, suffix, ctx, ctx_per_class, n_ctx, layout, eot, 0, C, C, L, feat_out, save_for_bwd, stream);
}

int mvlpt_text_fwd_grouped(void* h, const float* prefix, const float* suffix, const float* ctx, int n_ctx, const int32_t* layout,
                           const int32_t* eot, int G, int C, int L, float* feat_out, int save_for_bwd, mvlpt_stream_t stream) {
  Engine* E = (Engine*)h;
  if (!E || !prefix || !suffix || !ctx || !layout || !eot || !feat_out || G <= 0 || C <= 0 || L <= 0 || n_ctx <= 0)
    return fail(E, MVLPT_ERR_ARG, "text_fwd_grouped: null/invalid argument");
  if (G > 65535 || (int64_t)G * C > (int64_t)INT32_MAX / (L > 0 ? L : 1))
    return fail(E, MVLPT_ERR_ARG, "text_fwd_grouped: too many sequences");
  return text_fwd_impl(E, prefix, suffix, ctx, 0, n_ctx, layout, eot, G, C, G * C, L, feat_out, save_for_bwd, stream);
}

int mvlpt_text_fwd_ranged(void* h, const float* prefix, const float* suffix, const float* ctx, int n_ctx, const int32_t* layout,
                          const int32_t* eot, const int32_t* class_lo, const int32_t* class_hi, int G, int C, int L, float* feat_out,
                          int save_for_bwd, mvlpt_stream_t stream) {
  Engine* E = (Engine*)h;
  if (!E || !prefix || !suffix || !ctx || !layout || !eot || !class_lo || !class_hi || !feat_out || G <= 0 || C <= 0 || L <= 0 || n_ctx <= 0)
    return fail(E, MVLPT_ERR_ARG, "text_fwd_ranged: null/invalid argument");
  if (G > 65535) return fail(E, MVLPT_ERR_ARG, "text_fwd_ranged: too many groups");
  const int64_t S = build_range_table(class_lo, class_hi, G, C, E->t_range_host);
  if (S < 0) return fail(E, MVLPT_ERR_ARG, "text_fwd_ranged: a class range is not inside [0, C] or the ranges hold too many sequences");
  if (S == 0) return fail(E, MVLPT_ERR_ARG, "text_fwd_ranged: every range is empty");
  if (S > (int64_t)INT32_MAX / L) return fail(E, MVLPT_ERR_ARG, "text_fwd_ranged: too many sequences");
  return text_fwd_impl(E, prefix, suffix, ctx, 0, n_ctx, layout, eot, G, C, (int)S, L, feat_out, save_for_bwd, stream, true);
}

int mvlpt_text_encode_tokens(void* h, const int32_t* ids, int ld, int S, int L, float* feat_out, mvlpt_stream_t stream) {
  Engine* E = (Engine*)h;
  if (!E || !ids || !feat_out || S <= 0 || L <= 0 || ld < L) return fail(E, MVLPT_ERR_ARG, "text_encode_tokens: null/invalid argument");
  if (!E->tok_emb || E->vocab <= 0)
    return fail(E, MVLPT_ERR_STATE, "text_encode_tokens: token_embedding.weight is not loaded (mvlpt_load_frozen)");
  if (L < MVLPT_TEXT_MIN_L) return fail(E, MVLPT_ERR_ARG, "text_encode_tokens: L is below MVLPT_TEXT_MIN_L");
  if (L > E->arch.context_length) return fail(E, MVLPT_ERR_ARG, "text_encode_tokens: L exceeds context_length");
  if (S > 65535) return fail(E, MVLPT_ERR_ARG, "text_encode_tokens: more than 65535 sequences (the attention launches put the sequence on grid.y)");
  std::vector<int32_t>& t = E->t_ids_host;
  t.resize((size_t)S * L + S);
  int32_t* rows = t.data() + (size_t)S * L;
  for (int q = 0; q < S; ++q) {
    const int32_t* r = ids + (size_t)q * ld;
    int arg = 0;
    for (int i = 1; i < ld; ++i) if (r[i] > r[arg]) arg = i;
    if (arg >= L) return fail(E, MVLPT_ERR_ARG, "text_encode_tokens: the EOT position of sequence " + std::to_string(q) + " is not below L");
    for (int i = 0; i < L; ++i) {
      if (r[i] < 0 || r[i] >= E->vocab)
        return fail(E, MVLPT_ERR_ARG, "text_encode_tokens: token id outside [0, vocab) in sequence " + std::to_string(q));
      t[(size_t)q * L + i] = r[i];
    }
    rows[q] = q * L + arg;
  }
  return text_fwd_impl(E, nullptr, nullptr, nullptr, 0, 0, nullptr, nullptr, 0, S, S, L, feat_out, 0, stream, false, true);
}

int mvlpt_text_ensemble(const float* feats, int T, int C, int e, float* out, mvlpt_stream_t stream) {
  if (!feats || !out || T <= 0 || C <= 0 || e <= 0) { g_create_err = "text_ensemble: null/invalid argument"; return MVLPT_ERR_ARG; }
  const hipError_t rc = launch_ensemble_features(feats, out, T, C, e, (hipStream_t)stream);
  if (rc != hipSuccess) { g_create_err = std::string("text_ensemble: ") + hipGetErrorString(rc); return MVLPT_ERR_HIP; }
  return 0;
}

int mvlpt_text_workspace_bytes(void* h, int C_total, int L, int save_for_bwd, int64_t* out) {
  Engine* E = (Engine*)h;
  if (!E || !out || C_total <= 0 || L <= 2) return fail(E, MVLPT_ERR_ARG, "text_workspace_bytes: null/invalid argument");
  *out = (int64_t)text_ws_bytes(E, C_total, L, save_for_bwd != 0, text_exact(E), (size_t)C_total * (L - 2));
  return 0;
}

int mvlpt_text_bwd(void* h, const float* dfeat, float* dctx, mvlpt_stream_t stream) {
  Engine* E = (Engine*)h;
  if (!E || !dfeat || !dctx) return fail(E, MVLPT_ERR_ARG, "text_bwd: null argument");
  TowerState& st = E->ts;
  if (!st.valid || !st.saved) return fail(E, MVLPT_ERR_STATE, "text_bwd: call text_fwd(save_for_bwd=1) first");
  if (E->t_nctx <= 0) return fail(E, MVLPT_ERR_STATE, "text_bwd: the forward had no context tokens");
  hipStream_t s = (hipStream_t)stream;
  const MvlptArch& A = E->arch;
  const int C = E->tC, L = E->tL, dtw = A.text_width, e = A.embed_dim;
  const size_t T = (size_t)C * L;
  { ProfScope ps(E, s, PC_GLUE, 0, (double)T * dtw * 10.0);
    HIPCHK(E, launch_grad_scale(dfeat, (size_t)C * e, 64.0f, st.scale_dev, s));
    HIPCHK(E, launch_sgemm_bt(dfeat, E->tproj, E->deot32, C, dtw, e, st.scale_dev, s)); }
  { ProfScope ps(E, s, PC_GLUE, 0, (double)T * dtw * 4.0);
    HIPCHK(E, launch_zero(st.dx32, T * dtw * 4, s)); }
  if (!E->t_eot_last) return fail(E, MVLPT_ERR_STATE, "text_bwd: the forward did not keep the last block's activations");
  {
    const int l = st.layers - 1;
    const Block& Bk = E->txt.blocks[l];
    const int Ti = (int)T;
    const int xs = st.xs;
    const size_t X = xs ? 2 : 1;
    HIPCHK(E, ln_bwd(E, E->deot32, DT_F32, E->txo32, nullptr, 1, E->ln_final, nullptr, E->tdxc32, E->tdxc16, C, dtw, s, -1, xs));
    HIPCHK(E, gemm(E, xs ? EPI_GELUBWD_SPLIT : EPI_GELUBWD, E->tdxc16, Bk.pr.bw(), C, 4 * dtw, dtw, nullptr, E->tuc16, nullptr, E->tduc16, nullptr, s, -1, xs));
    HIPCHK(E, gemm(E, EPI_STORE32, E->tduc16, Bk.fc.bw(), C, dtw, 4 * dtw, nullptr, nullptr, nullptr, E->tdhc32, nullptr, s, -1, xs));
    HIPCHK(E, ln_bwd(E, E->tdhc32, DT_F32, E->txm32, nullptr, 1, Bk.ln2, E->tdxc32, E->tdxc32, E->tdxc16, C, dtw, s, -1, xs));
    HIPCHK(E, gemm(E, xs ? EPI_STORE_SPLIT : EPI_STORE16, E->tdxc16, Bk.o.bw(), C, dtw, dtw, nullptr, nullptr, nullptr, E->tdOc16, nullptr, s, -1, xs));
    { ProfScope ps(E, s, PC_GLUE, 0, (double)T * dtw * 2.0);
      HIPCHK(E, launch_zero(st.dO16, T * dtw * 2 * X, s));
      HIPCHK(E, launch_copy_rows(E->tdOc16, st.dO16, E->eot_rows, C, (int)(dtw * 2 * X), 1, s));
      HIPCHK(E, launch_copy_rows(E->tdxc32, st.dx32, E->eot_rows, C, dtw * 4, 1, s)); }
    if (xs) {
      if (int rc = attn32_bwd(E, st, l, s)) return rc;
    } else {
      AttnBwdArgs a{st.qkv[l], st.attn[l], st.dO16, st.lse[l], st.delta, st.dqkv16, st.N, st.L, st.H, 1};
      ProfScope ps(E, s, PC_ATTN_BWD, 7.0 * st.L * st.L * 64.0 * st.N * st.H, (double)T * dtw * 2.0 * 8.0);
      HIPCHK(E, launch_attn_bwd(E->dt, a, s));
    }
    HIPCHK(E, gemm(E, EPI_STORE32, st.dqkv16, Bk.qkv.bw(), Ti, dtw, 3 * dtw, nullptr, nullptr, nullptr, st.dh32, nullptr, s, -1, xs));
    HIPCHK(E, ln_bwd(E, st.dh32, DT_F32, st.x[2 * l], nullptr, 1, Bk.ln1, st.dx32, st.dx32, st.dx16, Ti, dtw, s, -1, xs));
  }
  for (int l = st.layers - 2; l >= 0; --l)
    if (int rc = block_bwd(E, E->txt, st, l, s)) return rc;
  { ProfScope ps(E, s, PC_GLUE, 0, (double)C * E->t_nctx * dtw * 4.0);
    if (E->t_ranged)
      HIPCHK(E, launch_gather_ctx_grad_ranged(st.dx32, E->ctx_pos, E->t_rlo, E->t_rstart, E->t_groups, L, dtw, E->t_nctx, dctx, st.scale_dev, s));
    else if (E->t_groups > 0)
      HIPCHK(E, launch_gather_ctx_grad_grouped(st.dx32, E->ctx_pos, E->t_groups, E->t_gC, L, dtw, E->t_nctx, dctx, st.scale_dev, s));
    else
      HIPCHK(E, launch_gather_ctx_grad(st.dx32, E->ctx_pos, C, L, dtw, E->t_nctx, E->t_per_class, dctx, st.scale_dev, s)); }
  return 0;
}

static int head_reserve(Engine* E, int B, int C) {
  const int e = E->arch.embed_dim;
  const size_t need = align256((size_t)B * e * 4) + align256((size_t)C * e * 4) + align256((size_t)B * 4) +
                      align256((size_t)C * 4) + 4096;
  HIPCHK(E, E->head_ws.reserve(need));
  Bump bp; bp.base = (char*)E->head_ws.p;
  E->imn = bp.take<float>((size_t)B * e); E->txn = bp.take<float>((size_t)C * e);
  E->inorm = bp.take<float>(B); E->tnorm = bp.take<float>(C);
  return 0;
}

int mvlpt_logits_fwd(void* h, const float* img, const float* txt, float scale, const int32_t* lo, const int32_t* hi, int B, int C,
                     float* logits, mvlpt_stream_t stream) {
  Engine* E = (Engine*)h;
  if (!E || !img || !txt || !logits || B <= 0 || C <= 0 || ((lo == nullptr) != (hi == nullptr)))
    return fail(E, MVLPT_ERR_ARG, "logits_fwd: null/invalid argument");
  hipStream_t s = (hipStream_t)stream;
  const int e = E->arch.embed_dim;
  E->hB = 0; E->h_grouped = false; E->h_ranged = false;
  if (int rc = head_reserve(E, B, C)) return rc;
  ProfScope ps(E, s, PC_HEAD, 2.0 * B * C * e, 4.0 * ((double)B * e + (double)C * e + (double)B * C));
  HIPCHK(E, launch_normalize_rows(img, E->imn, E->inorm, B, e, s));
  HIPCHK(E, launch_normalize_rows(txt, E->txn, E->tnorm, C, e, s));
  HIPCHK(E, launch_logits(E->imn, E->txn, scale, lo, hi, logits, B, C, e, s));
  E->hB = B; E->hC = C; E->h_scale = scale; E->h_lo = lo; E->h_hi = hi;
  return 0;
}

int mvlpt_logits_bwd(void* h, const float* dlogits, float* dimg, float* dtxt, mvlpt_stream_t stream) {
  Engine* E = (Engine*)h;
  if (!E || !dlogits) return fail(E, MVLPT_ERR_ARG, "logits_bwd: null argument");
  if (E->hB <= 0 || !E->imn || E->h_grouped || E->h_ranged) return fail(E, MVLPT_ERR_STATE, "logits_bwd: call logits_fwd first");
  hipStream_t s = (hipStream_t)stream;
  const int e = E->arch.embed_dim;
  ProfScope ps(E, s, PC_HEAD, 4.0 * E->hB * E->hC * e, 4.0 * ((double)E->hB * e + (double)E->hC * e + (double)E->hB * E->hC) * 2);
  HIPCHK(E, launch_logits_bwd(dlogits, E->imn, E->txn, E->inorm, E->tnorm, E->h_scale, E->h_lo, E->h_hi, dimg, dtxt, E->hB, E->hC, e, s));
  return 0;
}

int mvlpt_logits_grouped_fwd(void* h, const float* img, const float* txt, float scale, int G, int C, float* logits, mvlpt_stream_t stream) {
  Engine* E = (Engine*)h;
  if (!E || !img || !txt || !logits || G <= 0 || C <= 0 || G > 65535 || (int64_t)G * C > INT32_MAX)
    return fail(E, MVLPT_ERR_ARG, "logits_grouped_fwd: null/invalid argument");
  hipStream_t s = (hipStream_t)stream;
  const int e = E->arch.embed_dim;
  E->hB = 0; E->h_grouped = false; E->h_ranged = false;
  if (int rc = head_reserve(E, G, G * C)) return rc;
  ProfScope ps(E, s, PC_HEAD, 2.0 * G * C * e, 4.0 * ((double)G * e + (double)G * C * e + (double)G * C));
  HIPCHK(E, launch_normalize_rows(img, E->imn, E->inorm, G, e, s));
  HIPCHK(E, launch_normalize_rows(txt, E->txn, E->tnorm, G * C, e, s));
  HIPCHK(E, launch_logits_grouped(E->imn, E->txn, scale, logits, G, C, e, s));
  E->hB = G; E->hC = C; E->h_scale = scale; E->h_lo = E->h_hi = nullptr; E->h_grouped = true;
  return 0;
}

int mvlpt_logits_grouped_bwd(void* h, const float* dlogits, float* dtxt, mvlpt_stream_t stream) {
  Engine* E = (Engine*)h;
  if (!E || !dlogits || !dtxt) return fail(E, MVLPT_ERR_ARG, "logits_grouped_bwd: null argument");
  if (E->hB <= 0 || !E->imn || !E->h_grouped || E->h_ranged) return fail(E, MVLPT_ERR_STATE, "logits_grouped_bwd: call logits_grouped_fwd first");
  hipStream_t s = (hipStream_t)stream;
  const int e = E->arch.embed_dim;
  ProfScope ps(E, s, PC_HEAD, 4.0 * E->hB * E->hC * e, 4.0 * ((double)E->hB * e + 2.0 * E->hB * E->hC * e + (double)E->hB * E->hC));
  HIPCHK(E, launch_logits_grouped_bwd(dlogits, E->imn, E->txn, E->tnorm, E->h_scale, dtxt, E->hB, E->hC, e, s));
  return 0;
// ... 219 lines not shown
  return 0;
}
int mvlpt_op_layernorm_fwd_split(int out_dtype, const float* x, const float* gamma, const float* beta, void* y, int rows, int d,
                                 mvlpt_stream_t stream) {
  if (out_dtype == DT_F32) { g_create_err = "layernorm_fwd_split: 16-bit output only"; return MVLPT_ERR_ARG; }
  LnFwdArgs a{x, nullptr, 1, gamma, beta, y, rows, d};
  a.split = 1;
  OPCHK(launch_ln_fwd(out_dtype, a, (hipStream_t)stream));
  return 0;
}
int mvlpt_op_layernorm_bwd_split(int dtype, const void* dy, const float* x, const float* gamma, const float* resid, float* out32,
                                 void* out16, int rows, int d, mvlpt_stream_t stream) {
  LnBwdArgs a{dy, DT_F32, x, nullptr, 1, gamma, resid, out32, out16, rows, d};
  a.split = 1;
  OPCHK(launch_ln_bwd(dtype, a, (hipStream_t)stream));
  return 0;
}
int mvlpt_op_attention32_fwd(int dtype, const void* qkv, void* out, float* lse, int N, int L, int H, int causal, int q_rows,
                             mvlpt_stream_t stream) {
  Attn32Args a{qkv, out, lse, N, L, H, causal, q_rows};
#ifdef MVLPT_ATTN_TRACE
  const char* path = getenv("MVLPT_ATTN_TRACE_FILE");
  long long* tr = nullptr;
  const size_t tr_bytes = 8 * 256 * sizeof(long long);
  if (path) { OPCHK(hipMalloc(&tr, tr_bytes)); OPCHK(hipMemsetAsync(tr, 0, tr_bytes, (hipStream_t)stream)); a.trace = tr; }
#endif
  OPCHK(launch_attn32_fwd(dtype, a, (hipStream_t)stream));
#ifdef MVLPT_ATTN_TRACE
  if (path) {
    std::vector<long long> hbuf(8 * 256);
    OPCHK(hipStreamSynchronize((hipStream_t)stream));
    OPCHK(hipMemcpy(hbuf.data(), tr, tr_bytes, hipMemcpyDeviceToHost));
    if (FILE* f = fopen(path, "wb")) { fwrite(hbuf.data(), 1, tr_bytes, f); fclose(f); }
    (void)hipFree(tr);
  }
#endif
  return 0;
}
int mvlpt_op_attention32_bwd(int dtype, const void* qkv, const void* out, const void* dout, const float* lse, float* delta,
                             void* dqkv, int N, int L, int H, int causal, mvlpt_stream_t stream) {
  Attn32BwdArgs a{qkv, out, dout, lse, delta, dqkv, N, L, H, causal};
#ifdef MVLPT_ATTN_TRACE
  const char* path = getenv("MVLPT_ATTN_TRACE_FILE");
  long long* tr = nullptr;
  const size_t tr_bytes = 8 * 256 * sizeof(long long);
  if (path) { OPCHK(hipMalloc(&tr, tr_bytes)); OPCHK(hipMemsetAsync(tr, 0, tr_bytes, (hipStream_t)stream)); a.trace = tr; }
#endif
  OPCHK(launch_attn32_bwd(dtype, a, (hipStream_t)stream));
#ifdef MVLPT_ATTN_TRACE
  if (path) {
    std::vector<long long> hbuf(8 * 256);
    OPCHK(hipStreamSynchronize((hipStream_t)stream));
    OPCHK(hipMemcpy(hbuf.data(), tr, tr_bytes, hipMemcpyDeviceToHost));
    if (FILE* f = fopen(path, "wb")) { fwrite(hbuf.data(), 1, tr_bytes, f); fclose(f); }
    (void)hipFree(tr);
  }
#endif
  return 0;
}
int mvlpt_op_layernorm_fwd(int out_dtype, const float* x, const float* gamma, const float* beta, void* y, int rows, int d,
                           mvlpt_stream_t stream) {
  LnFwdArgs a{x, nullptr, 1, gamma, beta, y, rows, d};
  OPCHK(launch_ln_fwd(out_dtype, a, (hipStream_t)stream));
  return 0;
}
int mvlpt_op_layernorm_bwd(int dtype, const void* dy, const float* x, const float* gamma, const float* resid, float* out32,
                           void* out16, int rows, int d, mvlpt_stream_t stream) {
  LnBwdArgs a{dy, dtype, x, nullptr, 1, gamma, resid, out32, out16, rows, d};
  OPCHK(launch_ln_bwd(dtype, a, (hipStream_t)stream));
  return 0;
}
int mvlpt_op_attention_fwd(int dtype, const void* qkv, void* out, float* lse, int N, int L, int H, int causal,
                           mvlpt_stream_t stream) {
  AttnArgs a{qkv, out, lse, N, L, H, causal};
  OPCHK(launch_attn_fwd(dtype, a, (hipStream_t)stream));
  return 0;
}
int mvlpt_op_attention_bwd(int dtype, const void* qkv, const void* out, const void* dout, const float* lse, float* delta,
                           void* dqkv, int N, int L, int H, int causal, mvlpt_stream_t stream) {
  AttnBwdArgs a{qkv, out, dout, lse, delta, dqkv, N, L, H, causal};
  OPCHK(launch_attn_bwd(dtype, a, (hipStream_t)stream));
  return 0;
}
int mvlpt_op_cast(int dtype, const float* in, void* out, int64_t n, mvlpt_stream_t stream) {
  OPCHK(launch_cast_f32_to16(dtype, in, out, (size_t)n, nullptr, (hipStream_t)stream));
  return 0;
}
int mvlpt_op_assemble_prompts_grouped(const float* prefix, const float* suffix, const float* ctx, int n_ctx, const int32_t* layout,
                                      const float* pos, float* x, int G, int C, int L, int d, mvlpt_stream_t stream) {
  if (!prefix || !suffix || !ctx || !layout || !pos || !x || G <= 0 || C <= 0 || L <= n_ctx + 1 || n_ctx <= 0 || d <= 0) {
    g_create_err = "op_assemble_prompts_grouped: null/invalid argument"; return MVLPT_ERR_ARG; }
  OPCHK(launch_assemble_prompts_grouped(prefix, suffix, ctx, n_ctx, layout, pos, x, G, C, L, d, (hipStream_t)stream));
  return 0;
}
int mvlpt_op_gather_ctx_grad_grouped(const float* dx, const int32_t* ctx_pos, int G, int C, int L, int d, int n_ctx, float* dctx,
                                     mvlpt_stream_t stream) {
  if (!dx || !ctx_pos || !dctx || G <= 0 || C <= 0 || L <= 0 || n_ctx <= 0 || d <= 0) {
    g_create_err = "op_gather_ctx_grad_grouped: null/invalid argument"; return MVLPT_ERR_ARG; }
  OPCHK(launch_gather_ctx_grad_grouped(dx, ctx_pos, G, C, L, d, n_ctx, dctx, nullptr, (hipStream_t)stream));
  return 0;
}

static int op_range_table(const int32_t* class_lo, const int32_t* class_hi, int G, int C, std::vector<int32_t>& t, int32_t** dev, int* S) {
  const int64_t S64 = build_range_table(class_lo, class_hi, G, C, t);
  if (S64 <= 0) { g_create_err = "ranged op: a class range is not inside [0, C], or every range is empty"; return MVLPT_ERR_ARG; }
  *S = (int)S64;
  OPCHK(hipMalloc((void**)dev, t.size() * 4));
  hipError_t e = hipMemcpy(*dev, t.data(), t.size() * 4, hipMemcpyHostToDevice);
  if (e != hipSuccess) { (void)hipFree(*dev); *dev = nullptr; OPCHK(e); }
  return 0;
}
int mvlpt_op_assemble_prompts_ranged(const float* prefix, const float* suffix, const float* ctx, int n_ctx, const int32_t* layout,
                                     const float* pos, float* x, const int32_t* class_lo, const int32_t* class_hi, int G, int C, int L,
                                     int d, mvlpt_stream_t stream) {
  if (!prefix || !suffix || !ctx || !layout || !pos || !x || !class_lo || !class_hi || G <= 0 || C <= 0 || L <= n_ctx + 1 || n_ctx <= 0 ||
      d <= 0) {
    g_create_err = "op_assemble_prompts_ranged: null/invalid argument"; return MVLPT_ERR_ARG; }
  std::vector<int32_t> t; int32_t* dev = nullptr; int S = 0;
  if (int rc = op_range_table(class_lo, class_hi, G, C, t, &dev, &S)) return rc;
  hipError_t e = launch_assemble_prompts_ranged(prefix, suffix, ctx, n_ctx, layout, pos, x, dev + 2 * G + 1, dev + 2 * G + 1 + S, S, L, d,
                                                (hipStream_t)stream);
  if (e == hipSuccess) e = hipStreamSynchronize((hipStream_t)stream);
  (void)hipFree(dev);
  OPCHK(e);
  return 0;
}
int mvlpt_op_gather_ctx_grad_ranged(const float* dx, const int32_t* ctx_pos, const int32_t* class_lo, const int32_t* class_hi, int G, int C,
                                    int L, int d, int n_ctx, float* dctx, mvlpt_stream_t stream) {
  if (!dx || !ctx_pos || !dctx || !class_lo || !class_hi || G <= 0 || C <= 0 || L <= 0 || n_ctx <= 0 || d <= 0) {
    g_create_err = "op_gather_ctx_grad_ranged: null/invalid argument"; return MVLPT_ERR_ARG; }
  std::vector<int32_t> t; int32_t* dev = nullptr; int S = 0;
  if (int rc = op_range_table(class_lo, class_hi, G, C, t, &dev, &S)) return rc;
  hipError_t e = launch_gather_ctx_grad_ranged(dx, ctx_pos, dev, dev + G, G, L, d, n_ctx, dctx, nullptr, (hipStream_t)stream);
  if (e == hipSuccess) e = hipStreamSynchronize((hipStream_t)stream);
  (void)hipFree(dev);
  OPCHK(e);
  return 0;
}

int mvlpt_op_sgemm_bt(const float* A, const float* Bt, float* Cm, int M, int N, int K, const float* alpha_dev, mvlpt_stream_t stream) {
  if (!A || !Bt || !Cm) { g_create_err = "op_sgemm_bt: null argument"; return MVLPT_ERR_ARG; }
  OPCHK(launch_sgemm_bt(A, Bt, Cm, M, N, K, alpha_dev, (hipStream_t)stream));
  return 0;
}
int mvlpt_op_grad_scale(const float* v, int64_t n, float target, float* scale_dev, mvlpt_stream_t stream) {
  if (!v || !scale_dev || n <= 0 || !(target > 0.f)) { g_create_err = "op_grad_scale: null/invalid argument"; return MVLPT_ERR_ARG; }
  OPCHK(launch_grad_scale(v, (size_t)n, target, scale_dev, (hipStream_t)stream));
  return 0;
}
int mvlpt_op_reduce_prompt_rows(int dtype, float* dx32, void* dx16, int B, int L, int d, int row0, int n, float* out,
                                const float* scale_dev, int zero_after, int split16, const float* vmask, mvlpt_stream_t stream) {
  if (!dx32 || !out || B <= 0 || d <= 0 || n <= 0 || row0 < 0 || row0 + n > L || split16 < 0 || split16 > 2) {
    g_create_err = "op_reduce_prompt_rows: null/invalid argument"; return MVLPT_ERR_ARG; }
  OPCHK(launch_reduce_prompt_rows(dtype, dx32, dx16, B, L, d, row0, n, out, scale_dev, zero_after, (hipStream_t)stream, split16, vmask));
  return 0;
}
int mvlpt_op_gather_ctx_grad(const float* dx, const int32_t* ctx_pos, int C, int L, int d, int n_ctx, int per_class, float* dctx,
                             const float* scale_dev, mvlpt_stream_t stream) {
  if (!dx || !ctx_pos || !dctx || C <= 0 || L <= 0 || n_ctx <= 0 || d <= 0) {
    g_create_err = "op_gather_ctx_grad: null/invalid argument"; return MVLPT_ERR_ARG; }
  OPCHK(launch_gather_ctx_grad(dx, ctx_pos, C, L, d, n_ctx, per_class, dctx, scale_dev, (hipStream_t)stream));
  return 0;
}
int mvlpt_op_attention_bwd_cls(int dtype, const void* qkv, const void* o_cls, const void* do_cls, const float* lse, void* dqkv, int N,
                               int L, int H, mvlpt_stream_t stream) {
  if (!qkv || !o_cls || !do_cls || !lse || !dqkv) { g_create_err = "op_attention_bwd_cls: null argument"; return MVLPT_ERR_ARG; }
// ... 147 lines not shown
```

### mvlpt_amd/csrc/kernels.h

```cpp
#pragma once
#include "common.h"

namespace mvlpt {

int stream_cus(hipStream_t s);

enum GemmEpi {
  EPI_STORE16 = 0,
  EPI_GELU = 1,
  EPI_RESID32 = 2,
  EPI_GELUBWD = 3,
  EPI_STORE32 = 4,
  EPI_GELU_SPLIT = 5,
  EPI_GELUBWD_SPLIT = 6,
  EPI_STORE_SPLIT = 7,
  EPI_RESID32_LN = 8,
  EPI_STORE16_FOLD = 9, EPI_GELU_FOLD = 10, EPI_STORE_SPLIT_FOLD = 11, EPI_GELU_SPLIT_FOLD = 12,
  EPI_RESIDP_LN = 13,
};
constexpr int epi_base(int epi) {
  return epi == EPI_STORE16_FOLD ? EPI_STORE16 : epi == EPI_GELU_FOLD ? EPI_GELU : epi == EPI_STORE_SPLIT_FOLD ? EPI_STORE_SPLIT
         : epi == EPI_GELU_SPLIT_FOLD ? EPI_GELU_SPLIT : epi;
}
constexpr bool epi_folds(int epi) { return epi >= EPI_STORE16_FOLD && epi <= EPI_GELU_SPLIT_FOLD; }
// ... 3 lines not shown
  const void* Bt;
  int M, N, K;
  const float* bias;
  const void* aux;
  const float* resid;
  void* out;
  void* out2;
  int a_split = 0;
  int ldb = 0;
  int w8_exp = 0;
  int out_lo8 = 0;
  int lda = 0, ldo = 0;
  int xcd_order = 0;
  const float* ln_gamma = nullptr;
  void* ln_x16 = nullptr;
  int ln_split = 0;
  float* ln_part = nullptr;
  int ln_ntp = 0;
  const float* fold_part = nullptr;
  const float* fold_colsum = nullptr;
  int fold_ntp = 0, fold_nt = 0;
  const void* rp_hi_in = nullptr;
  const uint8_t* rp_lo_in = nullptr;
  uint8_t* rp_lo_out = nullptr;
#ifdef MVLPT_GEMM_TRACE
  long long* trace = nullptr;
#endif
};
int gemm_tile_n(int dtype, int epi, const GemmArgs& g, hipStream_t s);
enum GemmFamily {
  GEMM_FAM_BT_128x128_R2 = 1,
  GEMM_FAM_BT_128x128_R4 = 2,
  GEMM_FAM_BT_256x128_R3 = 3,
  GEMM_FAM_BT_256x256_R2 = 4,
  GEMM_FAM_PHASED = 5,
  GEMM_FAM_PC = 6,
  GEMM_FAM_PCP = 7,
};
struct GemmRoute { int family = 0, tile_m = 0, tile_n = 0, ring = 0; };
hipError_t gemm_route(int dtype, int epi, const GemmArgs& g, bool folded, hipStream_t s, GemmRoute* r);
hipError_t launch_gemm(int dtype, int epi, const GemmArgs& g, hipStream_t s, hipEvent_t ev_start = nullptr,
                       hipEvent_t ev_stop = nullptr);

hipError_t launch_sgemm_bt(const float* A, const float* Bt, float* C, int M, int N, int K, const float* alpha_dev, hipStream_t s);

struct LnFwdArgs {
  const float* x; const int32_t* row_idx; int row_mul;
  const float* gamma; const float* beta;
  void* y;
  int rows, d;
  int split = 0;
};
hipError_t launch_ln_fwd(int out_dtype, const LnFwdArgs& a, hipStream_t s);

struct LnBwdArgs {
  const void* dy;
  int dy_dtype;
  const float* x; const int32_t* row_idx; int row_mul;
  const float* gamma;
  const float* resid;
  float* out32;
  void* out16;
  int rows, d;
  int split = 0;
};
hipError_t launch_ln_bwd(int dtype, const LnBwdArgs& a, hipStream_t s);

struct AttnArgs {
  const void* qkv; void* out ; float* lse ;
  int N, L, H; int causal;
  int q_rows = 0;
  int flags = 0;
};
hipError_t launch_attn_fwd(int dtype, const AttnArgs& a, hipStream_t s, hipEvent_t ea = nullptr, hipEvent_t eb = nullptr);
struct AttnBwdArgs {
  const void* qkv; const void* out; const void* dout; const float* lse;
  float* delta ; void* dqkv ;
  int N, L, H; int causal;
};
hipError_t launch_attn_bwd(int dtype, const AttnBwdArgs& a, hipStream_t s);
int attn_max_len();
hipError_t launch_attn_bwd_cls(int dtype, const void* qkv, const void* o_cls, const void* do_cls, const float* lse, void* dqkv,
                               int N, int L, int H, hipStream_t s);
hipError_t launch_attn_fwd_stream(int dtype, const AttnArgs& a, hipStream_t s);
hipError_t launch_attn_bwd_stream(int dtype, const AttnBwdArgs& a, hipStream_t s);

struct Attn32Args {
  const void* qkv_split;
  void* out_split;
  float* lse;
  int N, L, H; int causal;
  int q_rows = 0;
  int out_lo8 = 0;
#ifdef MVLPT_ATTN_TRACE
  long long* trace = nullptr;
#endif
};
hipError_t launch_attn32_fwd(int dtype, const Attn32Args& a, hipStream_t s);
struct Attn32BwdArgs {
  const void* qkv_split; const void* out_split; const void* dout_split ; const float* lse;
  float* delta ; void* dqkv_split ;
  int N, L, H; int causal;
  int lo8 = 0;
#ifdef MVLPT_ATTN_TRACE
  long long* trace = nullptr;
#endif
};
hipError_t launch_attn32_bwd(int dtype, const Attn32BwdArgs& a, hipStream_t s);

struct PpDesc {
  int64_t offset;
  int32_t height, width;
  int32_t crop_top, crop_left, crop_h, crop_w;
  int32_t resize_h, resize_w;
  int32_t out_top, out_left;
  int32_t flip, reserved;
};
hipError_t launch_preprocess(const uint8_t* src, const PpDesc* descs_dev, int B, int max_crop_h, int ks_max, int out_h, int out_w,
                             int32_t* tables, size_t table_stride, uint8_t* tmp, size_t tmp_stride, const float* mean,
                             const float* stdv, void* out, int out_dtype, uint8_t* out_u8, hipStream_t s);

hipError_t launch_cast_f32_to16(int dtype, const float* in, void* out, size_t n, const float* scale_dev, hipStream_t s);
hipError_t launch_cast_f32_split(int dtype, const float* in, void* out, size_t rows, int d, const float* scale_dev, hipStream_t s, int lo8 = 0);
hipError_t launch_cast_any_to_f32(int in_dtype, const void* in, float* out, size_t n, hipStream_t s);
hipError_t launch_pack_weight(int dtype, const float* w, void* out, int rows, int cols, int ld_out, hipStream_t s);
hipError_t launch_pack_weight8(const float* w, uint8_t* out8, int rows, int cols, int transposed, int cols_out, size_t pitch_bytes,
                               const float* scale_dev, hipStream_t s);
hipError_t launch_pack_weight_t(int dtype, const float* w, void* out, int rows, int cols, hipStream_t s, int ld_out = 0);
hipError_t launch_patchify(int dtype, const void* image, int image_dtype, void* out, int B, int R, int P, int Kp, hipStream_t s);
hipError_t launch_assemble_tokens(const float* patch_emb, const float* cls, const float* pos, const float* g, const float* b,
                                  const float* vpt, int n_vpt, float* x, int B, int G2, int d, hipStream_t s,
                                  const float* vmask = nullptr );
hipError_t launch_assemble_tokens_packed(const float* patch_emb, const float* cls, const float* pos, const float* g, const float* b,
                                         void* hi, uint8_t* lo, float* part, int ntp, int B, int G2, int d, hipStream_t s);
hipError_t launch_overwrite_rows(const float* rows, int n, float* x, int B, int L, int d, hipStream_t s, const float* vmask = nullptr);
hipError_t launch_assemble_prompts(const float* prefix, const float* suffix, const float* ctx, int ctx_per_class, int n_ctx,
                                   const int32_t* layout, const float* pos, float* x, int C, int L, int d, hipStream_t s);
hipError_t launch_build_ctx_pos(const int32_t* layout, int32_t* ctx_pos, int C, int L, int n_ctx, hipStream_t s);
hipError_t launch_eot_rows(const int32_t* eot, int32_t* rows, int C, int L, hipStream_t s);
hipError_t launch_embed_tokens(const float* emb, const float* pos, const int32_t* ids, int ld, float* x, int S, int L, int d, hipStream_t s);
hipError_t launch_assemble_prompts_grouped(const float* prefix, const float* suffix, const float* ctx, int n_ctx, const int32_t* layout,
                                           const float* pos, float* x, int G, int C, int L, int d, hipStream_t s);
hipError_t launch_eot_rows_grouped(const int32_t* eot, int32_t* rows, int G, int C, int L, hipStream_t s);
hipError_t launch_copy_rows(const void* src, void* dst, const int32_t* idx, int rows, int row_bytes, int scatter, hipStream_t s);
hipError_t launch_copy_rows_strided(const void* src, void* dst, int rows, size_t src_pitch, size_t dst_pitch, int row_bytes, hipStream_t s);
hipError_t launch_reduce_prompt_rows(int dtype, float* dx32, void* dx16, int B, int L, int d, int row0, int n, float* out,
                                     const float* scale_dev, int zero_after, hipStream_t s, int split16 = 0, const float* vmask = nullptr);
hipError_t launch_gather_ctx_grad(const float* dx, const int32_t* ctx_pos, int C, int L, int d, int n_ctx, int per_class,
                                  float* dctx, const float* scale_dev, hipStream_t s);
hipError_t launch_gather_ctx_grad_grouped(const float* dx, const int32_t* ctx_pos, int G, int C, int L, int d, int n_ctx, float* dctx,
                                          const float* scale_dev, hipStream_t s);
hipError_t launch_assemble_prompts_ranged(const float* prefix, const float* suffix, const float* ctx, int n_ctx, const int32_t* layout,
                                          const float* pos, float* x, const int32_t* seq_cls, const int32_t* seq_grp, int S, int L, int d,
                                          hipStream_t s);
hipError_t launch_eot_rows_ranged(const int32_t* eot, int32_t* rows, const int32_t* seq_cls, int S, int L, hipStream_t s);
hipError_t launch_gather_ctx_grad_ranged(const float* dx, const int32_t* ctx_pos, const int32_t* lo, const int32_t* start, int G, int L,
                                         int d, int n_ctx, float* dctx, const float* scale_dev, hipStream_t s);
hipError_t launch_grad_scale(const float* v, size_t n, float target, float* scale_dev, hipStream_t s);
hipError_t launch_zero(void* p, size_t bytes, hipStream_t s);
hipError_t launch_checksum(const void* p, size_t bytes, unsigned long long* out, hipStream_t s);
hipError_t launch_fold_vectors(int dtype, const void* W16, int ld, const float* gamma, const float* beta, const float* b,
                               float* colsum, float* bias2, int N, int K, hipStream_t s);

hipError_t launch_fold_weight(const void* W16, int ld, const float* gamma, void* Wg16, int ldg, float* colsum, int N, int K, hipStream_t s);
hipError_t launch_respk_pack_rows(const float* x, void* hi, uint8_t* lo, float* part, int ntp, int rows, int d, hipStream_t s);
hipError_t launch_respk_unpack_rows(const void* hi, const uint8_t* lo, int row_mul, float* out, int rows, int d, hipStream_t s);

hipError_t launch_normalize_rows(const float* x, float* xn, float* norm, int rows, int d, hipStream_t s);
hipError_t launch_ensemble_features(const float* feats, float* out, int T, int C, int e, hipStream_t s);
hipError_t launch_logits(const float* imn, const float* txn, float scale, const int32_t* lo, const int32_t* hi,
                         float* logits, int B, int C, int e, hipStream_t s);
hipError_t launch_cross_entropy(const float* logits, const void* labels, int label_kind, int B, int C, float* row_loss,
                                float* loss, float* dlogits, float* ncorrect, hipStream_t s);
hipError_t launch_logits_bwd(const float* dlogits, const float* imn, const float* txn, const float* inorm, const float* tnorm,
                             float scale, const int32_t* lo, const int32_t* hi, float* dimg, float* dtxt,
                             int B, int C, int e, hipStream_t s);
hipError_t launch_logits_grouped(const float* imn, const float* txn, float scale, float* logits, int G, int C, int e, hipStream_t s);
hipError_t launch_logits_grouped_bwd(const float* dlogits, const float* imn, const float* txn, const float* tnorm, float scale, float* dtxt,
                                     int G, int C, int e, hipStream_t s);
hipError_t launch_logits_ranged(const float* imn, const float* txn, float scale, const int32_t* lo, const int32_t* start, float* logits,
                                int G, int C, int e, hipStream_t s);
hipError_t launch_logits_ranged_bwd(const float* dlogits, const float* imn, const float* txn, const float* inorm, const float* tnorm,
                                    float scale, const int32_t* lo, const int32_t* start, const int32_t* seq_grp, float* dimg, float* dtxt,
                                    int G, int S, int C, int e, hipStream_t s);

}
```

### mvlpt_amd/engine.py

```python
from __future__ import annotations

import ctypes as C
from typing import Dict, List, Optional, Tuple

import torch

from . import _lib
from ._lib import DT_BF16, DT_F16, DT_F32, lib
from .weights import ClipArch, arch_from_state_dict

_TORCH2DT = {torch.float32: DT_F32, torch.float16: DT_F16, torch.bfloat16: DT_BF16}
_DT2TORCH = {DT_F16: torch.float16, DT_BF16: torch.bfloat16, DT_F32: torch.float32}


def _ptr(t: Optional[torch.Tensor]):
    return None if t is None else C.c_void_p(t.data_ptr())


def _stream() -> C.c_void_p:
    return C.c_void_p(torch.cuda.current_stream().cuda_stream)


def _on_device(fn):
    import functools
# ... 628 lines not shown


def op_assemble_prompts(prefix, suffix, ctx, layout, pos, eot):
    C_, L = layout.shape
    d = prefix.shape[-1]
    n = 0 if ctx is None else ctx.shape[-2]
    x = torch.full((C_, L, d), float("nan"), device=prefix.device, dtype=torch.float32)
    ctx_pos = torch.full((C_, n), -1, device=prefix.device, dtype=torch.int32) if n else None
    rows = torch.full((C_,), -1, device=prefix.device, dtype=torch.int32)
    _lib.check(lib.mvlpt_op_assemble_prompts(_ptr(prefix.contiguous()), _ptr(suffix.contiguous()),
                                             _ptr(None if ctx is None else ctx.contiguous()), int(ctx is not None and ctx.dim() == 3), n,
                                             _ptr(layout.to(torch.int32).contiguous()), _ptr(pos.contiguous()),
                                             _ptr(eot.to(torch.int32).contiguous()), _ptr(x), _ptr(ctx_pos), _ptr(rows), C_, L, d,
                                             _stream()), None, "op_assemble_prompts")
    return x, ctx_pos, rows


def op_cast_mixed(x32: torch.Tensor, dtype) -> torch.Tensor:
    rows, d = x32.shape
    out = torch.zeros(rows, 2 * d, device=x32.device, dtype=dtype)
    _lib.check(lib.mvlpt_op_cast_mixed(_TORCH2DT[dtype], _ptr(x32.contiguous()), _ptr(out), rows, d, _stream()), None, "op_cast_mixed")
    return out


def op_pack_weight_mixed(w32: torch.Tensor, dtype, transposed=False):
    rows, cols = w32.shape
    R, K = (cols, rows) if transposed else (rows, cols)
    out = torch.zeros(R, K + K // 2, device=w32.device, dtype=dtype)
    e8 = C.c_int(0)
    _lib.check(lib.mvlpt_op_pack_weight_mixed(_TORCH2DT[dtype], _ptr(w32.contiguous()), rows, cols, int(transposed), _ptr(out),
                                              C.byref(e8), _stream()), None, "op_pack_weight_mixed")
    return out, e8.value


def op_gemm_mixed(A2, Wp, e8, epi=_lib.EPI_STORE32, bias=None, aux=None, resid=None, out2=False):
    dt = _TORCH2DT[A2.dtype]
    M, K = A2.shape[0], A2.shape[1] // 2
    N = Wp.shape[0]
    if epi in (_lib.EPI_RESID32, _lib.EPI_STORE32):
        out = torch.empty(M, N, device=A2.device, dtype=torch.float32)
    else:
        out = torch.zeros(M, 2 * N, device=A2.device, dtype=A2.dtype)
    o2 = torch.empty(M, N, device=A2.device, dtype=A2.dtype) if out2 else None
    _lib.check(lib.mvlpt_op_gemm_mixed(dt, epi, _ptr(A2.contiguous()), _ptr(Wp), Wp.shape[1], e8, M, N, K, _ptr(bias), _ptr(aux),
                                       _ptr(resid), _ptr(out), _ptr(o2), _stream()), None, "op_gemm_mixed")
    return (out, o2) if out2 else out


def op_layernorm_fwd_mixed(x, gamma, beta, out_dtype):
    rows, d = x.shape
    y = torch.zeros(rows, 2 * d, device=x.device, dtype=out_dtype)
    _lib.check(lib.mvlpt_op_layernorm_fwd_mixed(_TORCH2DT[out_dtype], _ptr(x), _ptr(gamma), _ptr(beta), _ptr(y), rows, d, _stream()),
               None, "op_layernorm_fwd_mixed")
    return y


def op_layernorm_bwd_mixed(dy32, x, gamma, dtype, resid=None):
    rows, d = x.shape
    out32 = torch.empty(rows, d, device=x.device, dtype=torch.float32)
    out16 = torch.zeros(rows, 2 * d, device=x.device, dtype=dtype)
    _lib.check(lib.mvlpt_op_layernorm_bwd_mixed(_TORCH2DT[dtype], _ptr(dy32), _ptr(x), _ptr(gamma), _ptr(resid), _ptr(out32),
                                                _ptr(out16), rows, d, _stream()), None, "op_layernorm_bwd_mixed")
    return out32, out16


def op_attention32_fwd_mixed(qkv_pair, N, L, H, causal, q_rows=0):
    dtype = qkv_pair.dtype
    out = torch.zeros(N * L, 2 * H * 64, device=qkv_pair.device, dtype=dtype)
    lse = torch.zeros(N * H * L, device=qkv_pair.device, dtype=torch.float32)
    _lib.check(lib.mvlpt_op_attention32_fwd_mixed(_TORCH2DT[dtype], _ptr(qkv_pair), _ptr(out), _ptr(lse), N, L, H, int(causal), q_rows,
                                                  _stream()), None, "op_attention32_fwd_mixed")
    return out, lse


def op_attention32_bwd_mixed(qkv_pair, out_mixed, dout_pair, lse, N, L, H, causal):
    dtype = out_mixed.dtype
    dqkv = torch.zeros(N * L, 6 * H * 64, device=qkv_pair.device, dtype=dtype)
    delta = torch.empty(N * H * L, device=qkv_pair.device, dtype=torch.float32)
    _lib.check(lib.mvlpt_op_attention32_bwd_mixed(_TORCH2DT[dtype], _ptr(qkv_pair), _ptr(out_mixed), _ptr(dout_pair), _ptr(lse),
                                                  _ptr(delta), _ptr(dqkv), N, L, H, int(causal), _stream()), None, "op_attention32_bwd_mixed")
    return dqkv


def op_layernorm_fwd_split(x, gamma, beta, out_dtype):
    rows, d = x.shape
    y = torch.empty(rows, 2 * d, device=x.device, dtype=out_dtype)
    _lib.check(lib.mvlpt_op_layernorm_fwd_split(_TORCH2DT[out_dtype], _ptr(x), _ptr(gamma), _ptr(beta), _ptr(y), rows, d, _stream()),
               None, "op_layernorm_fwd_split")
    return y


def op_layernorm_bwd_split(dy32, x, gamma, dtype, resid=None):
    rows, d = x.shape
    out32 = torch.empty(rows, d, device=x.device, dtype=torch.float32)
    out16 = torch.empty(rows, 2 * d, device=x.device, dtype=dtype)
    _lib.check(lib.mvlpt_op_layernorm_bwd_split(_TORCH2DT[dtype], _ptr(dy32), _ptr(x), _ptr(gamma), _ptr(resid), _ptr(out32),
                                                _ptr(out16), rows, d, _stream()), None, "op_layernorm_bwd_split")
    return out32, out16


def op_attention32_fwd_pair(qkv_pair, N, L, H, causal, q_rows=0):
    dtype = qkv_pair.dtype
    out = torch.zeros(N * L, 2 * H * 64, device=qkv_pair.device, dtype=dtype)
    lse = torch.zeros(N * H * L, device=qkv_pair.device, dtype=torch.float32)
    _lib.check(lib.mvlpt_op_attention32_fwd(_TORCH2DT[dtype], _ptr(qkv_pair), _ptr(out), _ptr(lse), N, L, H, int(causal), q_rows,
                                            _stream()), None, "op_attention32_fwd")
    return out, lse


def op_attention32_bwd_pair(qkv_pair, out_pair, dout_pair, lse, N, L, H, causal):
    dtype = out_pair.dtype
    dqkv = torch.empty(N * L, 6 * H * 64, device=qkv_pair.device, dtype=dtype)
    delta = torch.empty(N * H * L, device=qkv_pair.device, dtype=torch.float32)
    _lib.check(lib.mvlpt_op_attention32_bwd(_TORCH2DT[dtype], _ptr(qkv_pair), _ptr(out_pair), _ptr(dout_pair), _ptr(lse),
                                            _ptr(delta), _ptr(dqkv), N, L, H, int(causal), _stream()), None, "op_attention32_bwd")
    return dqkv


def op_attention32_fwd(qkv32, N, L, H, causal, dtype=torch.float16, q_rows=0):
    return op_attention32_fwd_pair(split_pair(qkv32, dtype), N, L, H, causal, q_rows)


def op_attention32_bwd(qkv32, out_pair, dout32, lse, N, L, H, causal):
    dtype = out_pair.dtype
    return op_attention32_bwd_pair(split_pair(qkv32, dtype), out_pair, split_pair(dout32, dtype), lse, N, L, H, causal)


def op_layernorm_fwd(x, gamma, beta, out_dtype):
    rows, d = x.shape
    y = torch.empty(rows, d, device=x.device, dtype=out_dtype)
    _lib.check(lib.mvlpt_op_layernorm_fwd(_TORCH2DT[out_dtype], _ptr(x), _ptr(gamma), _ptr(beta), _ptr(y), rows, d, _stream()),
               None, "op_layernorm_fwd")
    return y


def op_layernorm_bwd(dy, x, gamma, resid=None, want16=True):
    rows, d = x.shape
    out32 = torch.empty(rows, d, device=x.device, dtype=torch.float32)
    out16 = torch.empty(rows, d, device=x.device, dtype=dy.dtype) if want16 else None
    _lib.check(lib.mvlpt_op_layernorm_bwd(_TORCH2DT[dy.dtype], _ptr(dy), _ptr(x), _ptr(gamma), _ptr(resid), _ptr(out32),
                                          _ptr(out16), rows, d, _stream()), None, "op_layernorm_bwd")
    return out32, out16


def op_attention_fwd(qkv, N, L, H, causal, want_lse=True):
    out = torch.empty(N * L, H * 64, device=qkv.device, dtype=qkv.dtype)
    lse = torch.empty(N * H * L, device=qkv.device, dtype=torch.float32) if want_lse else None
    _lib.check(lib.mvlpt_op_attention_fwd(_TORCH2DT[qkv.dtype], _ptr(qkv), _ptr(out), _ptr(lse), N, L, H, int(causal), _stream()),
               None, "op_attention_fwd")
    return out, lse


def op_attention_bwd(qkv, out, dout, lse, N, L, H, causal):
    dqkv = torch.empty_like(qkv)
    delta = torch.empty(N * H * L, device=qkv.device, dtype=torch.float32)
    _lib.check(lib.mvlpt_op_attention_bwd(_TORCH2DT[qkv.dtype], _ptr(qkv), _ptr(out), _ptr(dout), _ptr(lse), _ptr(delta),
                                          _ptr(dqkv), N, L, H, int(causal), _stream()), None, "op_attention_bwd")
    return dqkv


def op_fold_vectors(W16: torch.Tensor, K: int, gamma, beta, b):
    N, ld = W16.shape
    cs = torch.empty(N, device=W16.device, dtype=torch.float32)
    b2 = torch.empty(N, device=W16.device, dtype=torch.float32)
    _lib.check(lib.mvlpt_op_fold_vectors(_TORCH2DT[W16.dtype], _ptr(W16), ld, _ptr(gamma), _ptr(beta), _ptr(b), _ptr(cs), _ptr(b2), N, K,
                                         _stream()), None, "op_fold_vectors")
    return cs, b2


def op_gemm_ln_producer(A, Bt, bias, resid, gamma, a_split=0, x16_split=0, ldb=0, w8_exp=0, ntp=8):
    dtype = A.dtype
    M = A.shape[0]
    K = A.shape[1] // (2 if a_split else 1)
    N = Bt.shape[0]
    out = torch.empty(M, N, device=A.device, dtype=torch.float32)
    x16 = torch.zeros(M, N * (2 if x16_split else 1), device=A.device, dtype=dtype)
    part = torch.zeros(M, ntp, 2, device=A.device, dtype=torch.float32)
    nt = C.c_int(0)
    _lib.check(lib.mvlpt_op_gemm_ln_producer(_TORCH2DT[dtype], _ptr(A.contiguous()), a_split, _ptr(Bt), ldb, w8_exp, M, N, K, _ptr(bias),
                                             _ptr(resid), _ptr(gamma), x16_split, _ptr(out), _ptr(x16), _ptr(part), ntp, C.byref(nt),
                                             _stream()), None, "op_gemm_ln_producer")
    return out, x16, part, nt.value


def op_fold_weight(W16: torch.Tensor, K: int, gamma):
    N, ld = W16.shape
    Wg = torch.empty(N, K, device=W16.device, dtype=torch.float16)
    cs = torch.empty(N, device=W16.device, dtype=torch.float32)
    _lib.check(lib.mvlpt_op_fold_weight(_ptr(W16), ld, _ptr(gamma), _ptr(Wg), K, _ptr(cs), N, K, _stream()), None, "op_fold_weight")
    return Wg, cs


def op_respk_pack(x: torch.Tensor, ntp: int = 0):
    rows, d = x.shape
    hi = torch.empty(rows, d, device=x.device, dtype=torch.float16)
    lo = torch.empty(rows, d, device=x.device, dtype=torch.int8)
    part = torch.full((rows, ntp, 2), float("nan"), device=x.device, dtype=torch.float32) if ntp else None
    _lib.check(lib.mvlpt_op_respk_pack(_ptr(x.contiguous()), _ptr(hi), _ptr(lo), _ptr(part), ntp, rows, d, _stream()), None, "op_respk_pack")
    return hi, lo, part


def op_assemble_packed(pe: torch.Tensor, cls: torch.Tensor, pos: torch.Tensor, g: torch.Tensor, b: torch.Tensor, batch: int, ntp: int = 6):
    d = pe.shape[1]
    G2 = pe.shape[0] // batch
    rows = batch * (1 + G2)
    hi = torch.empty(rows, d, device=pe.device, dtype=torch.float16)
    lo = torch.empty(rows, d, device=pe.device, dtype=torch.int8)
    part = torch.empty(rows, ntp, 2, device=pe.device, dtype=torch.float32)
    _lib.check(lib.mvlpt_op_assemble_packed(_ptr(pe), _ptr(cls), _ptr(pos), _ptr(g), _ptr(b), _ptr(hi), _ptr(lo), _ptr(part), ntp, batch, G2, d,
                                            _stream()), None, "op_assemble_packed")
    return hi, lo, part


def op_respk_unpack(hi: torch.Tensor, lo: torch.Tensor, row_mul: int = 1):
    rows, d = hi.shape[0] // row_mul, hi.shape[1]
    out = torch.empty(rows, d, device=hi.device, dtype=torch.float32)
    _lib.check(lib.mvlpt_op_respk_unpack(_ptr(hi), _ptr(lo), row_mul, _ptr(out), rows, d, _stream()), None, "op_respk_unpack")
    return out


def op_gemm_residp(A, Bt, bias, hi, lo, ldb=0, ntp=8, in_place=False):
    M, K = A.shape
    N = Bt.shape[0]
    ho = hi if in_place else torch.empty_like(hi)
    lo_o = lo if in_place else torch.empty_like(lo)
    part = torch.zeros(M, ntp, 2, device=A.device, dtype=torch.float32)
    nt = C.c_int(0)
    _lib.check(lib.mvlpt_op_gemm_residp(_ptr(A.contiguous()), _ptr(Bt), ldb, M, N, K, _ptr(bias), _ptr(hi), _ptr(lo), _ptr(ho), _ptr(lo_o),
                                        _ptr(part), ntp, C.byref(nt), _stream()), None, "op_gemm_residp")
    return ho, lo_o, part, nt.value


# ... 12 lines not shown
```

Baseline: 18730 images/sec.

## Compute text-tower last-layer attention only for EOT query rows

Adds single-query attention kernels, forward and backward, for the split-precision path. In the text tower's final layer they evaluate only the EOT row per prompt instead of running full causal attention, then gathering rows and scattering gradients. The backward kernel writes dQ/dK/dV directly and zeros the other rows, which removes the separate dO zero-fill and row scatter. It also adds a CLS-only forward kernel and op wrappers. The gain is limited to one layer of the text tower, and correctness depends on the zero-filling of non-query dqkv rows.

```diff
diff --git a/include/mvlpt_hip.h b/include/mvlpt_hip.h
--- a/include/mvlpt_hip.h
+++ b/include/mvlpt_hip.h
@@ -127,6 +127,14 @@
                            mvlpt_stream_t stream);
 int mvlpt_op_attention_bwd(int dtype, const void* qkv, const void* out, const void* dout, const float* lse, float* delta,
                            void* dqkv, int N, int L, int H, int causal, mvlpt_stream_t stream);
+int mvlpt_op_attention_fwd_rows(int dtype, const void* qkv, void* out, float* lse, int N, int L, int H, int causal, int q_rows,
+                                mvlpt_stream_t stream);
+int mvlpt_op_attention_fwd_cls(int dtype, const void* kv, int kv_ld, const void* q_cls, void* out_cls, float* lse, int N, int L, int H,
+                               mvlpt_stream_t stream);
+int mvlpt_op_attention32_fwd_q1(int dtype, const void* qkv, const int32_t* q_row, void* out_c, float* lse, int N, int L, int H, int out_lo8,
+                                mvlpt_stream_t stream);
+int mvlpt_op_attention32_bwd_q1(int dtype, const void* qkv, const int32_t* q_row, const void* o_c, const void* do_c, const float* lse,
+                                void* dqkv, int N, int L, int H, int lo8, mvlpt_stream_t stream);
 int mvlpt_op_cast(int dtype, const float* in, void* out, int64_t n, mvlpt_stream_t stream);
 int mvlpt_op_assemble_prompts_grouped(const float* prefix, const float* suffix, const float* ctx, int n_ctx, const int32_t* layout,
                                       const float* pos, float* x, int G, int C, int L, int d, mvlpt_stream_t stream);
diff --git a/mvlpt_amd/_lib.py b/mvlpt_amd/_lib.py
--- a/mvlpt_amd/_lib.py
+++ b/mvlpt_amd/_lib.py
@@ -94,6 +94,10 @@
     "mvlpt_op_layernorm_bwd": (_i, [_i, _vp, _vp, _vp, _vp, _vp, _vp, _i, _i, _vp]),
     "mvlpt_op_attention_fwd": (_i, [_i, _vp, _vp, _vp, _i, _i, _i, _i, _vp]),
     "mvlpt_op_attention_bwd": (_i, [_i, _vp, _vp, _vp, _vp, _vp, _vp, _i, _i, _i, _i, _vp]),
+    "mvlpt_op_attention_fwd_rows": (_i, [_i, _vp, _vp, _vp, _i, _i, _i, _i, _i, _vp]),
+    "mvlpt_op_attention_fwd_cls": (_i, [_i, _vp, _i, _vp, _vp, _vp, _i, _i, _i, _vp]),
+    "mvlpt_op_attention32_fwd_q1": (_i, [_i, _vp, _vp, _vp, _vp, _i, _i, _i, _i, _vp]),
+    "mvlpt_op_attention32_bwd_q1": (_i, [_i, _vp, _vp, _vp, _vp, _vp, _vp, _i, _i, _i, _i, _vp]),
     "mvlpt_op_cast": (_i, [_i, _vp, _vp, C.c_int64, _vp]),
     "mvlpt_op_assemble_prompts_grouped": (_i, [_vp, _vp, _vp, _i, _vp, _vp, _vp, _i, _i, _i, _i, _vp]),
     "mvlpt_op_gather_ctx_grad_grouped": (_i, [_vp, _vp, _i, _i, _i, _i, _i, _vp, _vp]),
diff --git a/mvlpt_amd/csrc/attention.hip b/mvlpt_amd/csrc/attention.hip
--- a/mvlpt_amd/csrc/attention.hip
+++ b/mvlpt_amd/csrc/attention.hip
@@ -586,6 +586,90 @@
   return hipGetLastError();
 }
 
+template <typename T>
+__global__ __launch_bounds__(256) void attn_fwd_cls_kernel(const T* __restrict__ kv, int kv_ld, const T* __restrict__ q_cls,
+                                                           T* __restrict__ out_cls, float* __restrict__ lse, int N, int L, int H) {
+  using v8 = typename Vec<T>::v8;
+  constexpr int U = 4;
+  constexpr float NEG = -1.0e30f;
+  const int lane = threadIdx.x & 63;
+  const int item = blockIdx.x * 4 + (threadIdx.x >> 6);
+  if (item >= N * H) return;
+  const int n = item / H, h = item % H, d = H * 64;
+  const int r = lane >> 3, c = lane & 7;
+  float q8[8];
+  {
+    const v8 qv = *(const v8*)(q_cls + (size_t)n * d + h * 64 + c * 8);
+#pragma unroll
+    for (int e = 0; e < 8; ++e) q8[e] = to_f32<T>(qv[e]) * (0.125f * 1.4426950408889634f);
+  }
+  const T* kbase = kv + (size_t)n * L * kv_ld + h * 64 + c * 8;
+  float m = NEG, sum = 0.f, acc[8];
+#pragma unroll
+  for (int e = 0; e < 8; ++e) acc[e] = 0.f;
+  for (int j0 = 0; j0 < L; j0 += 8 * U) {
+    v8 kk[U], vv[U];
+#pragma unroll
+    for (int u = 0; u < U; ++u) {
+      const int j = j0 + u * 8 + r;
+      const T* kp = kbase + (size_t)(j < L ? j : L - 1) * kv_ld;
+      kk[u] = __builtin_nontemporal_load((const v8*)kp);
+      vv[u] = __builtin_nontemporal_load((const v8*)(kp + d));
+    }
+    float sc[U], mn = m;
+#pragma unroll
+    for (int u = 0; u < U; ++u) {
+      float s = 0.f;
+#pragma unroll
+      for (int e = 0; e < 8; ++e) s = fmaf(q8[e], to_f32<T>(kk[u][e]), s);
+      s += __shfl_xor(s, 1, 64); s += __shfl_xor(s, 2, 64); s += __shfl_xor(s, 4, 64);
+      sc[u] = j0 + u * 8 + r < L ? s : NEG;
+      mn = fmaxf(mn, sc[u]);
+    }
+    const float alpha = __builtin_amdgcn_exp2f(m - mn);
+    m = mn;
+    sum *= alpha;
+#pragma unroll
+    for (int e = 0; e < 8; ++e) acc[e] *= alpha;
+#pragma unroll
+    for (int u = 0; u < U; ++u) {
+      const float p = j0 + u * 8 + r < L ? __builtin_amdgcn_exp2f(sc[u] - mn) : 0.f;
+      sum += p;
+#pragma unroll
+      for (int e = 0; e < 8; ++e) acc[e] = fmaf(p, to_f32<T>(vv[u][e]), acc[e]);
+    }
+  }
+  float mx = m;
+  mx = fmaxf(mx, __shfl_xor(mx, 8, 64)); mx = fmaxf(mx, __shfl_xor(mx, 16, 64)); mx = fmaxf(mx, __shfl_xor(mx, 32, 64));
+  const float w = __builtin_amdgcn_exp2f(m - mx);
+  sum *= w;
+  sum += __shfl_xor(sum, 8, 64); sum += __shfl_xor(sum, 16, 64); sum += __shfl_xor(sum, 32, 64);
+  const float inv = 1.0f / sum;
+  v8 o;
+#pragma unroll
+  for (int e = 0; e < 8; ++e) {
+    float a = acc[e] * w;
+    a += __shfl_xor(a, 8, 64); a += __shfl_xor(a, 16, 64); a += __shfl_xor(a, 32, 64);
+    o[e] = from_f32<T>(a * inv);
+  }
+  if (r == 0) *(v8*)(out_cls + (size_t)n * d + h * 64 + c * 8) = o;
+  if (lse && lane == 0) lse[((size_t)n * H + h) * L] = (mx + log2f(sum)) * 0.6931471805599453f;
+}
+
+hipError_t launch_attn_fwd_cls(int dtype, const void* kv, int kv_ld, const void* q_cls, void* out_cls, float* lse, int N, int L, int H,
+                               hipStream_t s) {
+  if (N <= 0 || L <= 0 || H <= 0 || kv_ld < 2 * H * 64 || (kv_ld & 7)) return hipErrorInvalidValue;
+  const int blocks = (N * H + 3) / 4;
+  if (dtype == DT_F16)
+    hipLaunchKernelGGL(attn_fwd_cls_kernel<f16>, dim3(blocks), dim3(256), 0, s, (const f16*)kv, kv_ld, (const f16*)q_cls, (f16*)out_cls,
+                       lse, N, L, H);
+  else if (dtype == DT_BF16)
+    hipLaunchKernelGGL(attn_fwd_cls_kernel<bf16>, dim3(blocks), dim3(256), 0, s, (const bf16*)kv, kv_ld, (const bf16*)q_cls,
+                       (bf16*)out_cls, lse, N, L, H);
+  else return hipErrorInvalidValue;
+  return hipGetLastError();
+}
+
 static thread_local hipEvent_t t_ev_a = nullptr, t_ev_b = nullptr;
 template <typename T, int NKT, bool CAUSAL>
 static hipError_t fwd_t(const AttnArgs& a, hipStream_t s) {
diff --git a/mvlpt_amd/csrc/attention32.hip b/mvlpt_amd/csrc/attention32.hip
--- a/mvlpt_amd/csrc/attention32.hip
+++ b/mvlpt_amd/csrc/attention32.hip
@@ -1200,6 +1200,210 @@
   return a.causal ? bwd_x<T, true, 4>(a, s) : bwd_x<T, false, 4>(a, s);
 }
 
+template <typename T>
+__global__ __launch_bounds__(256) void attn32_fwd_q1_kernel(const T* __restrict__ qkv, const int* __restrict__ q_row, T* __restrict__ out_c,
+                                                            float* __restrict__ lse, int N, int L, int H, int out_lo8) {
+  using v8 = typename Vec<T>::v8;
+  constexpr int U = 2;
+  constexpr float NEG = -1.0e30f;
+  constexpr float SC2 = SCALE * 1.4426950408889634f;
+  const int lane = threadIdx.x & 63;
+  const int item = blockIdx.x * 4 + (threadIdx.x >> 6);
+  if (item >= N * H) return;
+  const int n = item / H, h = item % H, d = H * 64;
+  const size_t ld = (size_t)6 * d, lo = (size_t)3 * d;
+  int qi = q_row[n] - n * L;
+  qi = qi < 0 ? 0 : (qi >= L ? L - 1 : qi);
+  const int r = lane >> 3, c = lane & 7;
+  const T* base = qkv + (size_t)n * L * ld + h * 64 + c * 8;
+  float qh[8], ql[8];
+  {
+    const T* qp = base + (size_t)qi * ld;
+    const v8 a = *(const v8*)qp, b = *(const v8*)(qp + lo);
+#pragma unroll
+    for (int e = 0; e < 8; ++e) { qh[e] = to_f32<T>(a[e]); ql[e] = to_f32<T>(b[e]); }
+  }
+  float m = NEG, sum = 0.f, acc[8];
+#pragma unroll
+  for (int e = 0; e < 8; ++e) acc[e] = 0.f;
+  for (int j0 = 0; j0 <= qi; j0 += 8 * U) {
+    v8 kh[U], kl[U], vh[U], vl[U];
+#pragma unroll
+    for (int u = 0; u < U; ++u) {
+      const int j = j0 + u * 8 + r;
+      const T* kp = base + (size_t)(j <= qi ? j : qi) * ld + d;
+      kh[u] = *(const v8*)kp; kl[u] = *(const v8*)(kp + lo);
+      vh[u] = *(const v8*)(kp + d); vl[u] = *(const v8*)(kp + d + lo);
+    }
+    float sc[U], mn = m;
+#pragma unroll
+    for (int u = 0; u < U; ++u) {
+      float s = 0.f;
+#pragma unroll
+      for (int e = 0; e < 8; ++e) {
+        const float a = to_f32<T>(kh[u][e]);
+        s = fmaf(qh[e], a, s); s = fmaf(qh[e], to_f32<T>(kl[u][e]), s); s = fmaf(ql[e], a, s);
+      }
+      s += __shfl_xor(s, 1, 64); s += __shfl_xor(s, 2, 64); s += __shfl_xor(s, 4, 64);
+      sc[u] = j0 + u * 8 + r <= qi ? s * SC2 : NEG;
+      mn = fmaxf(mn, sc[u]);
+    }
+    const float alpha = __builtin_amdgcn_exp2f(m - mn);
+    m = mn;
+    sum *= alpha;
+#pragma unroll
+    for (int e = 0; e < 8; ++e) acc[e] *= alpha;
+#pragma unroll
+    for (int u = 0; u < U; ++u) {
+      const float p = j0 + u * 8 + r <= qi ? __builtin_amdgcn_exp2f(sc[u] - mn) : 0.f;
+      sum += p;
+#pragma unroll
+      for (int e = 0; e < 8; ++e) acc[e] = fmaf(p, to_f32<T>(vh[u][e]) + to_f32<T>(vl[u][e]), acc[e]);
+    }
+  }
+  float mx = m;
+  mx = fmaxf(mx, __shfl_xor(mx, 8, 64)); mx = fmaxf(mx, __shfl_xor(mx, 16, 64)); mx = fmaxf(mx, __shfl_xor(mx, 32, 64));
+  const float w = __builtin_amdgcn_exp2f(m - mx);
+  sum *= w;
+  sum += __shfl_xor(sum, 8, 64); sum += __shfl_xor(sum, 16, 64); sum += __shfl_xor(sum, 32, 64);
+  const float inv = 1.0f / sum;
+  f32x4 o0, o1;
+#pragma unroll
+  for (int e = 0; e < 8; ++e) {
+    float a = acc[e] * w;
+    a += __shfl_xor(a, 8, 64); a += __shfl_xor(a, 16, 64); a += __shfl_xor(a, 32, 64);
+    if (e < 4) o0[e] = a * inv; else o1[e - 4] = a * inv;
+  }
+  if (r == 0) {
+    T* op = out_c + (size_t)n * 2 * d + h * 64 + c * 8;
+    store_pair4_m<T>(op, d, h * 64 + c * 8, o0, out_lo8);
+    store_pair4_m<T>(op + 4, d, h * 64 + c * 8 + 4, o1, out_lo8);
+  }
+  if (lse && lane == 0) lse[((size_t)n * H + h) * L + qi] = (mx + log2f(sum)) * 0.6931471805599453f;
+}
+
+__device__ __forceinline__ float q1_dot16(const float (&g)[16], const float (&a)[16]) {
+  float s = 0.f;
+#pragma unroll
+  for (int e = 0; e < 16; ++e) s = fmaf(g[e], a[e], s);
+  s += __shfl_xor(s, 1, 64); s += __shfl_xor(s, 2, 64);
+  return s;
+}
+template <typename T>
+__global__ __launch_bounds__(256) void attn32_bwd_q1_kernel(const T* __restrict__ qkv, const int* __restrict__ q_row,
+                                                            const T* __restrict__ o_c, const T* __restrict__ do_c,
+                                                            const float* __restrict__ lse, T* __restrict__ dqkv, int N, int L, int H, int lo8) {
+  using v8 = typename Vec<T>::v8;
+  __shared__ float red[4][64];
+  const int n = blockIdx.x / H, h = blockIdx.x % H, d = H * 64, tid = threadIdx.x;
+  const size_t ld = (size_t)6 * d, lo = (size_t)3 * d;
+  int qi = q_row[n] - n * L;
+  qi = qi < 0 ? 0 : (qi >= L ? L - 1 : qi);
+  const int lane = tid & 63, wave = tid >> 6, kg = lane >> 2, ch = lane & 3;
+  const T* base = qkv + (size_t)n * L * ld + h * 64 + ch * 16;
+  T* gbase = dqkv + (size_t)n * L * ld;
+  const int col = h * 64 + ch * 16;
+  float qh[16], ql[16], q16[16], g16[16], o16[16], dqa[16];
+  {
+    const T* qp = base + (size_t)qi * ld;
+    const T* gp = do_c + (size_t)n * 2 * d + col;
+    const T* op = o_c + (size_t)n * 2 * d + col;
+#pragma unroll
+    for (int k = 0; k < 2; ++k) {
+      const v8 a = *(const v8*)(qp + 8 * k), b = *(const v8*)(qp + lo + 8 * k);
+      const v8 ga = *(const v8*)(gp + 8 * k), gb = *(const v8*)(gp + d + 8 * k);
+#pragma unroll
+      for (int e = 0; e < 8; ++e) {
+        qh[8 * k + e] = to_f32<T>(a[e]); ql[8 * k + e] = to_f32<T>(b[e]);
+        q16[8 * k + e] = qh[8 * k + e] + ql[8 * k + e];
+        g16[8 * k + e] = to_f32<T>(ga[e]) + to_f32<T>(gb[e]);
+        dqa[8 * k + e] = 0.f;
+      }
+    }
+#pragma unroll
+    for (int k = 0; k < 4; ++k) {
+      const f32x4 o = load_pair4_m<T>(op + 4 * k, d, col + 4 * k, lo8);
+#pragma unroll
+      for (int e = 0; e < 4; ++e) o16[4 * k + e] = o[e];
+    }
+  }
+  const float delta = q1_dot16(g16, o16);
+  const float l0 = lse[((size_t)n * H + h) * L + qi];
+  const f32x4 zero = {0.f, 0.f, 0.f, 0.f};
+  for (int j0 = wave * 16; j0 < L; j0 += 64) {
+    const int j = j0 + kg;
+    const bool live = j <= qi;
+    const T* kp = base + (size_t)(live ? j : qi) * ld + d;
+    float k16[16], v16[16], sdot = 0.f;
+#pragma unroll
+    for (int k = 0; k < 2; ++k) {
+      const v8 a = *(const v8*)(kp + 8 * k), b = *(const v8*)(kp + lo + 8 * k);
+      const v8 va = *(const v8*)(kp + d + 8 * k), vb = *(const v8*)(kp + d + lo + 8 * k);
+#pragma unroll
+      for (int e = 0; e < 8; ++e) {
+        const float x = to_f32<T>(a[e]), y = to_f32<T>(b[e]);
+        sdot = fmaf(qh[8 * k + e], x, sdot); sdot = fmaf(qh[8 * k + e], y, sdot); sdot = fmaf(ql[8 * k + e], x, sdot);
+        k16[8 * k + e] = x + y;
+        v16[8 * k + e] = to_f32<T>(va[e]) + to_f32<T>(vb[e]);
+      }
+    }
+    const float dp = q1_dot16(g16, v16);
+    sdot += __shfl_xor(sdot, 1, 64); sdot += __shfl_xor(sdot, 2, 64);
+    const float pj = live ? __expf(sdot * SCALE - l0) : 0.f;
+    const float ds = pj * (dp - delta) * SCALE;
+#pragma unroll
+    for (int e = 0; e < 16; ++e) dqa[e] = fmaf(ds, k16[e], dqa[e]);
+    if (j < L) {
+      T* gp = gbase + (size_t)j * ld + col;
+#pragma unroll
+      for (int k = 0; k < 4; ++k) {
+        if (j != qi) store_pair4_m<T>(gp + 4 * k, lo, col + 4 * k, zero, lo8);
+        store_pair4_m<T>(gp + d + 4 * k, lo, d + col + 4 * k,
+                         f32x4{ds * q16[4 * k], ds * q16[4 * k + 1], ds * q16[4 * k + 2], ds * q16[4 * k + 3]}, lo8);
+        store_pair4_m<T>(gp + 2 * d + 4 * k, lo, 2 * d + col + 4 * k,
+                         f32x4{pj * g16[4 * k], pj * g16[4 * k + 1], pj * g16[4 * k + 2], pj * g16[4 * k + 3]}, lo8);
+      }
+    }
+  }
+#pragma unroll
+  for (int e = 0; e < 16; ++e) {
+    float v = dqa[e];
+    v += __shfl_xor(v, 4, 64); v += __shfl_xor(v, 8, 64); v += __shfl_xor(v, 16, 64); v += __shfl_xor(v, 32, 64);
+    if (kg == 0) red[wave][ch * 16 + e] = v;
+  }
+  __syncthreads();
+  if (tid < 16) {
+    f32x4 v;
+#pragma unroll
+    for (int e = 0; e < 4; ++e) v[e] = (red[0][tid * 4 + e] + red[1][tid * 4 + e]) + (red[2][tid * 4 + e] + red[3][tid * 4 + e]);
+    store_pair4_m<T>(gbase + (size_t)qi * ld + h * 64 + tid * 4, lo, h * 64 + tid * 4, v, lo8);
+  }
+}
+
+hipError_t launch_attn32_fwd_q1(int dtype, const void* qkv_split, const int* q_row, void* out_c, float* lse, int N, int L, int H, int out_lo8,
+                                hipStream_t s) {
+  if (N <= 0 || L <= 0 || H <= 0 || !qkv_split || !q_row || !out_c) return hipErrorInvalidValue;
+  const int blocks = (N * H + 3) / 4;
+  if (dtype == DT_F16)
+    hipLaunchKernelGGL(attn32_fwd_q1_kernel<f16>, dim3(blocks), dim3(256), 0, s, (const f16*)qkv_split, q_row, (f16*)out_c, lse, N, L, H, out_lo8);
+  else if (dtype == DT_BF16)
+    hipLaunchKernelGGL(attn32_fwd_q1_kernel<bf16>, dim3(blocks), dim3(256), 0, s, (const bf16*)qkv_split, q_row, (bf16*)out_c, lse, N, L, H, out_lo8);
+  else return hipErrorInvalidValue;
+  return hipGetLastError();
+}
+hipError_t launch_attn32_bwd_q1(int dtype, const void* qkv_split, const int* q_row, const void* o_c, const void* do_c, const float* lse,
+                                void* dqkv_split, int N, int L, int H, int lo8, hipStream_t s) {
+  if (N <= 0 || L <= 0 || H <= 0 || !qkv_split || !q_row || !o_c || !do_c || !lse || !dqkv_split) return hipErrorInvalidValue;
+  if (dtype == DT_F16)
+    hipLaunchKernelGGL(attn32_bwd_q1_kernel<f16>, dim3(N * H), dim3(256), 0, s, (const f16*)qkv_split, q_row, (const f16*)o_c, (const f16*)do_c,
+                       lse, (f16*)dqkv_split, N, L, H, lo8);
+  else if (dtype == DT_BF16)
+    hipLaunchKernelGGL(attn32_bwd_q1_kernel<bf16>, dim3(N * H), dim3(256), 0, s, (const bf16*)qkv_split, q_row, (const bf16*)o_c,
+                       (const bf16*)do_c, lse, (bf16*)dqkv_split, N, L, H, lo8);
+  else return hipErrorInvalidValue;
+  return hipGetLastError();
+}
+
 hipError_t launch_attn32_fwd(int dtype, const Attn32Args& a, hipStream_t s) {
   if (a.L <= 0 || a.N <= 0 || a.H <= 0 || !a.qkv_split || !a.out_split) return hipErrorInvalidValue;
   if (dtype == DT_F16) return fwd_t<f16>(a, s);
diff --git a/mvlpt_amd/csrc/engine.hip b/mvlpt_amd/csrc/engine.hip
--- a/mvlpt_amd/csrc/engine.hip
+++ b/mvlpt_amd/csrc/engine.hip
@@ -138,7 +138,7 @@
   DevBuf vis_ws, txt_ws, head_ws, ce_ws, tmp, pp_ws;
   TowerState vs, ts;
   int vB = 0, v_nvpt = 0, v_ndeep = 0; float* cls32 = nullptr; float* dcls32 = nullptr;
-  float* xc32 = nullptr; void *ac16 = nullptr, *hc16 = nullptr, *gc16 = nullptr;
+  float* xc32 = nullptr; void *ac16 = nullptr, *hc16 = nullptr, *gc16 = nullptr, *qc16 = nullptr;
   bool v_cls_last = false; float *xcm32 = nullptr, *xco32 = nullptr, *dxc32 = nullptr, *dhc32 = nullptr;
   void *uc16 = nullptr, *duc16 = nullptr, *dxc16 = nullptr, *dOc16 = nullptr;
   int tC = 0, tL = 0, t_nctx = 0, t_per_class = 0; int32_t* eot_rows = nullptr; int32_t* ctx_pos = nullptr;
@@ -811,7 +811,7 @@
   const size_t X = exact ? 2 : 1;
   const size_t npatch = (size_t)B * G2;
   size_t need = tower_bytes(E->vis, B, Lv, save, exact) + align256(npatch * E->Kp * 2) + align256(npatch * dv * 4) +
-                7 * align256((size_t)B * dv * 4) + 4 * align256((size_t)B * dv * 2 * X) + 3 * align256((size_t)B * dv * 8 * X) + 4096;
+                7 * align256((size_t)B * dv * 4) + 5 * align256((size_t)B * dv * 2 * X) + 3 * align256((size_t)B * dv * 8 * X) + 4096;
   E->vs.valid = false;
   HIPCHK(E, E->vis_ws.reserve(need));
   Bump bp; bp.base = (char*)E->vis_ws.p; bp.cap = E->vis_ws.cap;
@@ -821,6 +821,7 @@
   E->dcls32 = bp.take<float>((size_t)B * dv);
   E->xc32 = bp.take<float>((size_t)B * dv);
   E->ac16 = bp.take_bytes((size_t)B * dv * 2 * X); E->hc16 = bp.take_bytes((size_t)B * dv * 2 * X);
+  E->qc16 = bp.take_bytes((size_t)B * dv * 2 * X);
   E->gc16 = bp.take_bytes((size_t)B * dv * 4 * 2 * X);
   E->xcm32 = bp.take<float>((size_t)B * dv); E->xco32 = bp.take<float>((size_t)B * dv);
   E->dxc32 = bp.take<float>((size_t)B * dv); E->dhc32 = bp.take<float>((size_t)B * dv);
@@ -896,26 +897,46 @@
     float* xout = save ? E->xco32 : E->xc32;
     E->v_cls_last = save;
     const int xs = st.xs;
+    const bool kv_only = !xs && !save;
     Fold fq;
     if (ln1_ready) fq = fold_consumer(st, 0, Bk.qkv);
     else HIPCHK(E, ln_fwd(E, E->dt, xin, nullptr, 1, Bk.ln1, st.h16, T, dv, s, xs));
     if (packed) fq.fold_colsum = Bk.qkv.fold_sg;
-    HIPCHK(E, gemm(E, xs ? EPI_STORE_SPLIT : EPI_STORE16, packed ? xhi : st.h16, packed ? Bk.qkv.fwg() : Bk.qkv.fw(), T, 3 * dv, dv,
-                   ln1_ready ? Bk.qkv.fold_b : Bk.qkv.b, nullptr, nullptr, st.qkv[l], nullptr, s, -1, xs, ln1_ready ? &fq : nullptr));
-    dbg_ck(E, st.qkv[l], (size_t)T * 3 * dv * 2 * X, s);
-    if (xs) {
-      if (save) HIPCHK(E, launch_zero(st.attn[l], (size_t)T * dv * 4, s));
-      if (int rc = attn32_fwd(E, st, l, 1, s)) return rc;
+    if (kv_only) {
+      { ProfScope ps(E, s, PC_GLUE, 0, (double)B * dv * 7.0);
+        if (packed) HIPCHK(E, launch_respk_unpack_rows(xhi, xlo, Lv, E->xc32, B, dv, s));
+        else HIPCHK(E, launch_copy_rows_strided(xin, E->xc32, B, (size_t)Lv * dv * 4, (size_t)dv * 4, dv * 4, s)); }
+      dbg_ck(E, E->xc32, (size_t)B * dv * 4, s);
+      WRef wkv = packed ? Bk.qkv.fwg() : Bk.qkv.fw();
+      wkv.p = (const char*)wkv.p + (size_t)dv * wkv.ld * 2;
+      if (ln1_ready) fq.fold_colsum += dv;
+      const float* bkv = ln1_ready ? Bk.qkv.fold_b : Bk.qkv.b;
+      HIPCHK(E, gemm(E, EPI_STORE16, packed ? xhi : st.h16, wkv, T, 2 * dv, dv, bkv ? bkv + dv : nullptr, nullptr, nullptr,
+                     st.qkv[l], nullptr, s, -1, 0, ln1_ready ? &fq : nullptr));
+      dbg_ck(E, st.qkv[l], (size_t)T * 2 * dv * 2, s);
+      HIPCHK(E, ln_fwd(E, E->dt, E->xc32, nullptr, 1, Bk.ln1, E->hc16, B, dv, s));
+      HIPCHK(E, gemm(E, EPI_STORE16, E->hc16, Bk.qkv.fw(), B, dv, dv, Bk.qkv.b, nullptr, nullptr, E->qc16, nullptr, s));
+      dbg_ck(E, E->qc16, (size_t)B * dv * 2, s);
+      { ProfScope ps(E, s, PC_ATTN_FWD, 4.0 * st.L * 64.0 * st.N * st.H, (double)T * dv * 2.0 * 2.0 + (double)B * dv * 2.0 * 2.0);
+        HIPCHK(E, launch_attn_fwd_cls(E->dt, st.qkv[l], 2 * dv, E->qc16, E->ac16, nullptr, st.N, st.L, st.H, s)); }
     } else {
-      AttnArgs a{st.qkv[l], st.attn[l], save ? st.lse[l] : nullptr, st.N, st.L, st.H, 0, 1};
-      ProfScope ps(E, s, PC_ATTN_FWD, 4.0 * st.L * 64.0 * st.N * st.H, (double)T * dv * 2.0 * 2.0);
-      HIPCHK(E, launch_attn_fwd(E->dt, a, s));
+      HIPCHK(E, gemm(E, xs ? EPI_STORE_SPLIT : EPI_STORE16, st.h16, Bk.qkv.fw(), T, 3 * dv, dv, ln1_ready ? Bk.qkv.fold_b : Bk.qkv.b, nullptr, nullptr,
+                     st.qkv[l], nullptr, s, -1, xs, ln1_ready ? &fq : nullptr));
+      dbg_ck(E, st.qkv[l], (size_t)T * 3 * dv * 2 * X, s);
+      if (xs) {
+        if (save) HIPCHK(E, launch_zero(st.attn[l], (size_t)T * dv * 4, s));
+        if (int rc = attn32_fwd(E, st, l, 1, s)) return rc;
+      } else {
+        AttnArgs a{st.qkv[l], st.attn[l], save ? st.lse[l] : nullptr, st.N, st.L, st.H, 0, 1};
+        ProfScope ps(E, s, PC_ATTN_FWD, 4.0 * st.L * 64.0 * st.N * st.H, (double)T * dv * 2.0 * 2.0);
+        HIPCHK(E, launch_attn_fwd(E->dt, a, s));
+      }
+      { ProfScope ps(E, s, PC_GLUE, 0, (double)B * dv * 12.0);
+        HIPCHK(E, launch_copy_rows_strided(st.attn[l], E->ac16, B, (size_t)Lv * dv * 2 * X, (size_t)dv * 2 * X, (int)(dv * 2 * X), s));
+        HIPCHK(E, launch_copy_rows_strided(xin, E->xc32, B, (size_t)Lv * dv * 4, (size_t)dv * 4, dv * 4, s)); }
+      dbg_ck(E, E->xc32, (size_t)B * dv * 4, s);
     }
-    { ProfScope ps(E, s, PC_GLUE, 0, (double)B * dv * 12.0);
-      HIPCHK(E, launch_copy_rows_strided(st.attn[l], E->ac16, B, (size_t)Lv * dv * 2 * X, (size_t)dv * 2 * X, (int)(dv * 2 * X), s));
-      if (packed) HIPCHK(E, launch_respk_unpack_rows(xhi, xlo, Lv, E->xc32, B, dv, s));
-      else HIPCHK(E, launch_copy_rows_strided(xin, E->xc32, B, (size_t)Lv * dv * 4, (size_t)dv * 4, dv * 4, s)); }
-    dbg_ck(E, E->ac16, (size_t)B * dv * 2 * X, s); dbg_ck(E, E->xc32, (size_t)B * dv * 4, s);
+    dbg_ck(E, E->ac16, (size_t)B * dv * 2 * X, s);
     HIPCHK(E, gemm(E, EPI_RESID32, E->ac16, Bk.o.fw(), B, dv, dv, Bk.o.b, nullptr, E->xc32, xmid, nullptr, s, -1, xs));
     HIPCHK(E, ln_fwd(E, E->dt, xmid, nullptr, 1, Bk.ln2, E->hc16, B, dv, s, xs));
     HIPCHK(E, gemm(E, xs ? EPI_GELU_SPLIT : EPI_GELU, E->hc16, Bk.fc.fw(), B, 4 * dv, dv, Bk.fc.b, nullptr, nullptr, E->gc16, save ? E->uc16 : nullptr, s, -1, xs));
@@ -1100,14 +1121,16 @@
     HIPCHK(E, gemm(E, xs ? EPI_STORE_SPLIT : EPI_STORE16, st.h16, Bk.qkv.fw(), T, 3 * dtw, dtw, ln1_ready ? Bk.qkv.fold_b : Bk.qkv.b, nullptr, nullptr, st.qkv[l], nullptr, s, -1, xs,
                    ln1_ready ? &fq : nullptr));
     if (xs) {
-      if (int rc = attn32_fwd(E, st, l, 0, s)) return rc;
+      ProfScope ps(E, s, PC_ATTN_FWD, 2.0 * st.L * 64.0 * st.N * st.H, (double)T * dtw * 2.0 * 2.0 * 2.0 * 0.5);
+      HIPCHK(E, launch_attn32_fwd_q1(E->dt, st.qkv[l], E->eot_rows, E->tac16, save ? st.lse[l] : nullptr, st.N, st.L, st.H, xs == 2 ? 1 : 0, s));
     } else {
       AttnArgs a{st.qkv[l], st.attn[l], save ? st.lse[l] : nullptr, st.N, st.L, st.H, 1};
-      ProfScope ps(E, s, PC_ATTN_FWD, 2.0 * st.L * st.L * 64.0 * st.N * st.H, (double)T * dtw * 2.0 * 4.0);
-      HIPCHK(E, launch_attn_fwd(E->dt, a, s));
+      { ProfScope ps(E, s, PC_ATTN_FWD, 2.0 * st.L * st.L * 64.0 * st.N * st.H, (double)T * dtw * 2.0 * 4.0);
+        HIPCHK(E, launch_attn_fwd(E->dt, a, s)); }
+      ProfScope ps(E, s, PC_GLUE, 0, (double)C * dtw * 4.0);
+      HIPCHK(E, launch_copy_rows(st.attn[l], E->tac16, E->eot_rows, C, (int)(dtw * 2 * X), 0, s));
     }
-    { ProfScope ps(E, s, PC_GLUE, 0, (double)C * dtw * 12.0);
-      HIPCHK(E, launch_copy_rows(st.attn[l], E->tac16, E->eot_rows, C, (int)(dtw * 2 * X), 0, s));
+    { ProfScope ps(E, s, PC_GLUE, 0, (double)C * dtw * 8.0);
       HIPCHK(E, launch_copy_rows(xin, E->txc32, E->eot_rows, C, dtw * 4, 0, s)); }
     HIPCHK(E, gemm(E, EPI_RESID32, E->tac16, Bk.o.fw(), C, dtw, dtw, Bk.o.b, nullptr, E->txc32, E->txm32, nullptr, s, -1, xs));
     HIPCHK(E, ln_fwd(E, E->dt, E->txm32, nullptr, 1, Bk.ln2, E->thc16, C, dtw, s, xs));
@@ -1220,13 +1243,15 @@
     HIPCHK(E, gemm(E, EPI_STORE32, E->tduc16, Bk.fc.bw(), C, dtw, 4 * dtw, nullptr, nullptr, nullptr, E->tdhc32, nullptr, s, -1, xs));
     HIPCHK(E, ln_bwd(E, E->tdhc32, DT_F32, E->txm32, nullptr, 1, Bk.ln2, E->tdxc32, E->tdxc32, E->tdxc16, C, dtw, s, -1, xs));
     HIPCHK(E, gemm(E, xs ? EPI_STORE_SPLIT : EPI_STORE16, E->tdxc16, Bk.o.bw(), C, dtw, dtw, nullptr, nullptr, nullptr, E->tdOc16, nullptr, s, -1, xs));
-    { ProfScope ps(E, s, PC_GLUE, 0, (double)T * dtw * 2.0);
-      HIPCHK(E, launch_zero(st.dO16, T * dtw * 2 * X, s));
-      HIPCHK(E, launch_copy_rows(E->tdOc16, st.dO16, E->eot_rows, C, (int)(dtw * 2 * X), 1, s));
+    { ProfScope ps(E, s, PC_GLUE, 0, (double)C * dtw * 8.0);
       HIPCHK(E, launch_copy_rows(E->tdxc32, st.dx32, E->eot_rows, C, dtw * 4, 1, s)); }
     if (xs) {
-      if (int rc = attn32_bwd(E, st, l, s)) return rc;
+      ProfScope ps(E, s, PC_ATTN_BWD, 5.0 * st.L * 64.0 * st.N * st.H, (double)T * dtw * 2.0 * (2.0 + 3.0 * (xs == 2 ? 1.5 : 2.0)));
+      HIPCHK(E, launch_attn32_bwd_q1(E->dt, st.qkv[l], E->eot_rows, E->tac16, E->tdOc16, st.lse[l], st.dqkv16, st.N, st.L, st.H, xs == 2 ? 1 : 0, s));
     } else {
+      { ProfScope ps(E, s, PC_GLUE, 0, (double)T * dtw * 2.0);
+        HIPCHK(E, launch_zero(st.dO16, T * dtw * 2, s));
+        HIPCHK(E, launch_copy_rows(E->tdOc16, st.dO16, E->eot_rows, C, dtw * 2, 1, s)); }
       AttnBwdArgs a{st.qkv[l], st.attn[l], st.dO16, st.lse[l], st.delta, st.dqkv16, st.N, st.L, st.H, 1};
       ProfScope ps(E, s, PC_ATTN_BWD, 7.0 * st.L * st.L * 64.0 * st.N * st.H, (double)T * dtw * 2.0 * 8.0);
       HIPCHK(E, launch_attn_bwd(E->dt, a, s));
@@ -1612,6 +1637,28 @@
   OPCHK(launch_attn_bwd(dtype, a, (hipStream_t)stream));
   return 0;
 }
+int mvlpt_op_attention_fwd_rows(int dtype, const void* qkv, void* out, float* lse, int N, int L, int H, int causal, int q_rows,
+                                mvlpt_stream_t stream) {
+  AttnArgs a{qkv, out, lse, N, L, H, causal, q_rows};
+  OPCHK(launch_attn_fwd(dtype, a, (hipStream_t)stream));
+  return 0;
+}
+int mvlpt_op_attention_fwd_cls(int dtype, const void* kv, int kv_ld, const void* q_cls, void* out_cls, float* lse, int N, int L, int H,
+                               mvlpt_stream_t stream) {
+  if (!kv || !q_cls || !out_cls) return fail(nullptr, MVLPT_ERR_ARG, "op_attention_fwd_cls: null argument");
+  OPCHK(launch_attn_fwd_cls(dtype, kv, kv_ld, q_cls, out_cls, lse, N, L, H, (hipStream_t)stream));
+  return 0;
+}
+int mvlpt_op_attention32_fwd_q1(int dtype, const void* qkv, const int32_t* q_row, void* out_c, float* lse, int N, int L, int H, int out_lo8,
+                                mvlpt_stream_t stream) {
+  OPCHK(launch_attn32_fwd_q1(dtype, qkv, q_row, out_c, lse, N, L, H, out_lo8, (hipStream_t)stream));
+  return 0;
+}
+int mvlpt_op_attention32_bwd_q1(int dtype, const void* qkv, const int32_t* q_row, const void* o_c, const void* do_c, const float* lse,
+                                void* dqkv, int N, int L, int H, int lo8, mvlpt_stream_t stream) {
+  OPCHK(launch_attn32_bwd_q1(dtype, qkv, q_row, o_c, do_c, lse, dqkv, N, L, H, lo8, (hipStream_t)stream));
+  return 0;
+}
 int mvlpt_op_cast(int dtype, const float* in, void* out, int64_t n, mvlpt_stream_t stream) {
   OPCHK(launch_cast_f32_to16(dtype, in, out, (size_t)n, nullptr, (hipStream_t)stream));
   return 0;
diff --git a/mvlpt_amd/csrc/kernels.h b/mvlpt_amd/csrc/kernels.h
--- a/mvlpt_amd/csrc/kernels.h
+++ b/mvlpt_amd/csrc/kernels.h
@@ -109,6 +109,8 @@
 int attn_max_len();
 hipError_t launch_attn_bwd_cls(int dtype, const void* qkv, const void* o_cls, const void* do_cls, const float* lse, void* dqkv,
                                int N, int L, int H, hipStream_t s);
+hipError_t launch_attn_fwd_cls(int dtype, const void* kv, int kv_ld, const void* q_cls, void* out_cls, float* lse, int N, int L, int H,
+                               hipStream_t s);
 hipError_t launch_attn_fwd_stream(int dtype, const AttnArgs& a, hipStream_t s);
 hipError_t launch_attn_bwd_stream(int dtype, const AttnBwdArgs& a, hipStream_t s);
 
@@ -134,6 +136,10 @@
 #endif
 };
 hipError_t launch_attn32_bwd(int dtype, const Attn32BwdArgs& a, hipStream_t s);
+hipError_t launch_attn32_fwd_q1(int dtype, const void* qkv_split, const int* q_row, void* out_c, float* lse, int N, int L, int H, int out_lo8,
+                                hipStream_t s);
+hipError_t launch_attn32_bwd_q1(int dtype, const void* qkv_split, const int* q_row, const void* o_c, const void* do_c, const float* lse,
+                                void* dqkv_split, int N, int L, int H, int lo8, hipStream_t s);
 
 struct PpDesc {
   int64_t offset;
diff --git a/mvlpt_amd/engine.py b/mvlpt_amd/engine.py
--- a/mvlpt_amd/engine.py
+++ b/mvlpt_amd/engine.py
@@ -734,6 +734,23 @@
     return dqkv
 
 
+def op_attention32_fwd_q1(qkv_pair, q_row, N, L, H, mixed=False, want_lse=True, fill=float("nan")):
+    dtype = qkv_pair.dtype
+    out = torch.zeros(N, 2 * H * 64, device=qkv_pair.device, dtype=dtype)
+    lse = torch.full((N * H * L,), fill, device=qkv_pair.device, dtype=torch.float32) if want_lse else None
+    _lib.check(lib.mvlpt_op_attention32_fwd_q1(_TORCH2DT[dtype], _ptr(qkv_pair), _ptr(q_row), _ptr(out), _ptr(lse), N, L, H, int(mixed),
+                                               _stream()), None, "op_attention32_fwd_q1")
+    return out, lse
+
+
+def op_attention32_bwd_q1(qkv_pair, q_row, o_c, do_c, lse, N, L, H, mixed=False, fill=float("nan")):
+    dtype = qkv_pair.dtype
+    dqkv = torch.full((N * L, 6 * H * 64), fill, device=qkv_pair.device, dtype=dtype)
+    _lib.check(lib.mvlpt_op_attention32_bwd_q1(_TORCH2DT[dtype], _ptr(qkv_pair), _ptr(q_row), _ptr(o_c), _ptr(do_c), _ptr(lse), _ptr(dqkv),
+                                               N, L, H, int(mixed), _stream()), None, "op_attention32_bwd_q1")
+    return dqkv
+
+
 def op_layernorm_fwd_split(x, gamma, beta, out_dtype):
     rows, d = x.shape
     y = torch.empty(rows, 2 * d, device=x.device, dtype=out_dtype)
@@ -800,6 +817,23 @@
     lse = torch.empty(N * H * L, device=qkv.device, dtype=torch.float32) if want_lse else None
     _lib.check(lib.mvlpt_op_attention_fwd(_TORCH2DT[qkv.dtype], _ptr(qkv), _ptr(out), _ptr(lse), N, L, H, int(causal), _stream()),
                None, "op_attention_fwd")
+    return out, lse
+
+
+def op_attention_fwd_rows(qkv, N, L, H, causal, q_rows, fill=float("nan")):
+    out = torch.full((N * L, H * 64), fill, device=qkv.device, dtype=qkv.dtype)
+    lse = torch.full((N * H * L,), fill, device=qkv.device, dtype=torch.float32)
+    _lib.check(lib.mvlpt_op_attention_fwd_rows(_TORCH2DT[qkv.dtype], _ptr(qkv), _ptr(out), _ptr(lse), N, L, H, int(causal), q_rows,
+                                               _stream()), None, "op_attention_fwd_rows")
+    return out, lse
+
+
+def op_attention_fwd_cls(kv, q_cls, N, L, H, want_lse=True, fill=float("nan")):
+    assert kv.stride(1) == 1 and kv.shape[0] == N * L
+    out = torch.full((N, H * 64), fill, device=kv.device, dtype=kv.dtype)
+    lse = torch.full((N * H * L,), fill, device=kv.device, dtype=torch.float32) if want_lse else None
+    _lib.check(lib.mvlpt_op_attention_fwd_cls(_TORCH2DT[kv.dtype], _ptr(kv), kv.stride(0), _ptr(q_cls.contiguous()), _ptr(out), _ptr(lse),
+                                              N, L, H, _stream()), None, "op_attention_fwd_cls")
     return out, lse
 
 
```

Measured after the change: 18890 images/sec (median of 6 runs). Within noise of the previous version (+0.9%).
